# BUTSpeechFIT/huggingface_asr

Hardware: AMD Instinct MI355X
Metric: audio-seconds/sec encoder fwd+CTC, E-Branchformer-base (higher is better)
Workload: dtype bf16; 1 GPU; E-Branchformer-base enc+CTC (relative-pos), 32x10s 16kHz clips/GPU: fbank+CMVN -> conv2d sub -> 16 layers -> CTC head -> CTC loss (the batch-independent projection of the relative-position table, 0.2 % of the FLOPs, is cached across steps); per_gpu_batch=32, frames=1000, encoder_frames=250, parallelism=replicas x1 (no exchange step), steps_in_flight=4, wide_tiles=True, hw_queues=8

## Files before the change

huggingface_asr_amd/_lib.py:

```python
from __future__ import annotations

import ctypes as C
import os

_HERE = os.path.dirname(os.path.abspath(__file__))
LIB_PATH = os.environ.get("HFASR_HIP_LIB") or os.path.join(_HERE, "libhfasr_hip.so")

vp, i32, i64, f32, f64, sz = C.c_void_p, C.c_int, C.c_long, C.c_float, C.c_double, C.c_size_t


class EbfConfig(C.Structure):
    _fields_ = [(n, i32) for n in ("B", "T", "F", "d", "H", "I", "L", "V", "C1", "C2", "K", "stride", "pad",
                                   "is_causal", "pos_type", "csgu_kernel", "merge_kernel", "csgu_act", "use_macaron")] + \
               [("ln_eps", f32), ("logits_f32", i32), ("logits_ld", i32), ("branch_overlap", i32), ("extra_layers", i32), ("layer_mixing", i32), ("csgu_linear", i32),
                ("context_mode", i32), ("gate_blk", i32), ("ln_fold", i32), ("wide_tiles", i32)]


class LnRedDesc(C.Structure):
    _fields_ = [("partial", vp), ("nblk", i32), ("d", i32), ("dgamma", vp), ("dbeta", vp), ("kind", i32)]


class Gpt2Config(C.Structure):
    _fields_ = [("d", i32), ("H", i32), ("L", i32), ("V", i32), ("eps", f32), ("step_form", i32), ("act", i32)]


GLOBAL_SLOTS, LAYER_SLOTS = 24, 64

SIGNATURES = {
    "mi_gemm_bf16": [vp, i64, vp, i64, vp, i32, vp, i64, i32, vp, i64, f32, i32, i32, i32, i32, i32, i32, vp],
    "mi_conv2d_cl_bf16": [vp, vp, vp, vp] + [i32] * 13 + [vp],
    "mi_gemm_bf16_v": [vp, i64, vp, i64, vp, i32, vp, i64, i32, vp, i64, f32, i32, i32, i32, i32, i32, i32, i32, vp],
    "mi_conv2d_cl_bf16_v": [vp, vp, vp, vp] + [i32] * 14 + [vp],
    "mi_conv2d_first_gelu": [vp, vp, vp, vp] + [i32] * 10 + [vp],
    "mi_conv2d_first_geo": [vp, vp, vp, vp] + [i32] * 13 + [vp],
    "mi_conv2d_first_gated_gelu": [vp, vp, vp, vp, vp, vp] + [i32] * 10 + [vp],
    "mi_conv2d_cl_geo_bf16": [vp, vp, vp, vp] + [i32] * 15 + [vp],
    "mi_gated_act_bf16": [vp, i64, vp, i64, vp, i64, i32, i32, i32, i32, i32, i32, vp],
    "mi_im2col_cl_geo_bf16": [vp, vp] + [i32] * 12 + [vp],
    "mi_col2im_cl_bf16": [vp, vp] + [i32] * 13 + [vp],
    "mi_gated_act_bwd_bf16": [vp, i64, vp, i64, vp, i64, vp, i64, vp, i64, i32, i32, i32, i32, i32, vp],
    "mi_conv2d_first_wgrad": [vp, vp, vp, vp] + [i32] * 12 + [vp, vp],
    "mi_gemm_lnfold_bf16": [vp, i64, vp, i64, vp, vp, vp, i32, f32, vp, i64, i32, i32, i32, i32, vp],
    "mi_gemm_resid_stats_f32": [vp, i64, vp, i64, vp, vp, i64, vp, i64, f32, vp, i64, vp, i32, i32, i32, vp],
    "mi_layernorm_fold": [vp, i64, vp, i32, vp, vp, f32, vp, i64, vp, i64, vp, i32, i32, vp],
    "mi_layernorm_chain": [vp, i64, vp, i32, vp, vp, f32, vp, i64, vp, vp, f32, vp, i64, vp, i64, vp, vp, vp, i64, i32, i32, vp],
    "mi_cast_f32_bf16": [vp, i64, vp, i64, i32, i32, vp],
    "mi_rotary_bf16": [vp, i64, vp, i64, vp, vp, i32, i32, i32, i32, vp],
    "mi_attention_bf16": [vp, i64, vp, i64, vp, i64, i32, vp, i64, vp, vp, vp, vp, i64, i32, i32, i32, i32, f32, i32, vp],
    "mi_attention_qkv_bf16": [vp, i64, vp, i64, vp, i64, vp, i64, vp, vp, vp, vp, i64, i32, i32, i32, i64, i32, i32, f32, i32, vp],
    "mi_attention_qkv_bf16_v": [vp, i64, vp, i64, vp, i64, vp, i64, vp, vp, vp, vp, i64, i32, i32, i32, i64, i32, i32, f32, i32, i32, vp],
    "mi_attention_x_lse_bf16": [vp, i64, vp, i64, vp, i64, vp, vp, i64, vp, i32, i32, i32, i32, i32, f32, i32, f32, C.c_uint, C.c_uint, vp],
    "mi_attention_x_bwd_probs": [vp, i64, vp, i64, vp, i64, vp, vp, i64, vp, i64, vp, vp, vp, i64, vp, i64, i32, i32, i32, i32, i32, f32, i32, f32, C.c_uint, C.c_uint, vp],
    "mi_attention_qkv_lse_bf16": [vp, i64, vp, i64, vp, i64, vp, i64, vp, vp, vp, vp, i64, vp, i32, i32, i32, i32, f32, i32, f32, C.c_uint, C.c_uint, vp],
    "mi_attention_qkv_bwd_probs": [vp, i64, vp, i64, vp, i64, vp, i64, vp, vp, vp, vp, i64, vp, i64, vp, vp, vp, i64, vp, i64, i32,
                                   vp, i64, vp, vp, vp, vp, i64, i32, i32, i32, i32, f32, i32, f32, C.c_uint, C.c_uint, i32, vp],
    "mi_attention_qkv_bwd_fused": [vp, vp, vp, i64, vp, vp, i64, vp, i64, vp, vp, vp, vp, i64, vp, sz, i32, i32, i32, i32, f32, vp],
    "mi_row_stats_bf16": [vp, i64, i32, f32, vp, i32, vp],
    "mi_csgu_bf16": [vp, i64, vp, vp, vp, vp, vp, vp, i64, i32, i32, i32, i32, i32, i32, i32, vp],
    "mi_dwconv_residual_bf16": [vp, i64, vp, vp, vp, i64, i32, i32, i32, i32, i32, vp],
    "mi_fbank_f64": [vp, i64, vp, i32, vp, vp, vp, vp, vp, vp, i32, i32, i32, f64, f64, vp],
    "mi_trim_zeros_pad_f32": [vp, i64, vp, i32, i32, i32, vp, i64, i32, vp, vp, vp, vp],
    "mi_cmvn_utterance": [vp, vp, i32, i32, i32, i32, i32, f32, vp],
    "mi_cmvn_global": [vp, i64, i32, vp, vp, vp],
    "mi_row_lse": [vp, i64, i32, i32, vp, i32, vp],
    "mi_gemm_lse_f32": [vp, i64, vp, i64, vp, vp, i64, vp, vp, i32, i32, i32, vp],
    "mi_gemm_lse_workspace_floats": [i32, i32],
    "mi_row_argmax": [vp, i64, i32, i32, vp, i32, vp],
    "mi_ctc_collapse": [vp, i32, i32, vp, i32, i64, vp, i32, vp, vp, vp],
    "mi_ctc_greedy": [vp, i64, i64, i32, i32, i32, i32, vp, i32, i64, vp, vp, i32, vp, vp, vp],
    "mi_ctc_beam_workspace_bytes": [i32, i32, i32],
    "mi_ctc_beam_cut": [vp, i64, i64, i32, i32, i32, i32, vp, i32, i32, vp, vp, vp, vp, vp],
    "mi_ctc_beam_walk": [vp, i64, i64, i32, i32, i32, i32, vp, i32, i64, i32, i32, i32, vp, vp, vp, vp, vp, sz, vp, i32, vp, vp, vp, vp],
    "mi_ctc_beam_stream_state_bytes": [i32, i32, i32],
    "mi_ctc_beam_stream_reset": [vp, sz, i32, i32, i32, vp],
    "mi_ctc_beam_stream_walk": [vp, i64, i64, i32, i32, i32, i32, vp, i32, i64, i32, i32, i32, vp, vp, vp, vp, vp, sz, i32, i32, vp, vp, vp, vp, vp, i32, vp, vp, vp, vp],
    "mi_ctc_align_workspace_bytes": [i32, i32, i32],
    "mi_ctc_align": [vp, i64, i64, i32, vp, i32, vp, i32, vp, i32, i32, i32, vp, sz, vp, vp, vp, vp, vp, vp, vp],
    "mi_gemm_argmax_workspace_floats": [i32, i32],
    "mi_gemm_argmax_bf16": [vp, i64, vp, i64, vp, vp, vp, i32, i32, i32, vp],
    "mi_gemm_ce_f32": [vp, i64, vp, i64, vp, vp, vp, vp, vp, vp, vp, i32, i32, i32, vp],
    "mi_gemm_ce_bwd_bf16": [vp, i64, vp, i64, vp, vp, vp, vp, vp, i64, i32, i32, i32, vp],
    "mi_ctc_loss_fwd": [vp, i64, i64, i32, vp, i32, vp, i32, vp, i32, i32, i32, i32, vp, vp, vp, vp],
    "mi_ctc_prefix_prepare": [vp, i64, i64, i32, vp, i32, i32, i32, i32, i32, vp, vp, vp, vp],
    "mi_ctc_prefix_score": [vp, i32, i32, i32, i32, i32, vp, vp, i64, i32, vp, vp, vp, vp],
    "mi_embed_tokens": [vp, vp, f32, vp, i32, i32, i32, i32, i32, vp, vp],
    "mi_ce_label_smoothing": [vp, i64, vp, i32, i32, i32, i32, f32, vp, vp, vp],
    "mi_whisper_logmel": [vp, i64, vp, i32, vp, vp, vp, i32, i32, vp, vp, vp, vp],
    "mi_transpose_cast_bct_btc": [vp, vp, i32, i32, i32, vp],
    "mi_add_positions": [vp, vp, vp, i32, i32, i32, vp],
    "mi_transpose_bf16": [vp, i64, vp, i64, i32, i32, i32, vp],
    "mi_transpose_many_bf16": [vp, i32, vp],
    "mi_colsum": [vp, i64, i32, i32, i32, vp, vp, vp],
    "mi_act_fwd_bf16": [vp, i64, vp, i64, i32, i32, i32, vp],
    "mi_act_bwd_bf16": [vp, i64, vp, i64, vp, i64, i32, i32, i32, vp],
    "mi_act_dropout_fwd_bf16": [vp, i64, vp, i64, i32, i32, i32, f32, C.c_uint, C.c_uint, vp],
    "mi_act_dropout_bwd_bf16": [vp, i64, vp, i64, vp, i64, i32, i32, i32, f32, C.c_uint, C.c_uint, vp],
    "mi_layernorm_bwd_workspace_floats": [i32],
    "mi_layernorm_bwd": [vp, i64, i32, vp, f32, vp, i64, i32, vp, i64, i32, i32, vp, vp, vp, i32, i32, vp],
    "mi_layernorm_bwd_partial": [vp, i64, i32, vp, f32, vp, i64, i32, vp, i64, i32, i32, vp, vp, i32, i32, vp],
    "mi_layernorm_bwd_dual_partial": [vp, i64, i32, f32, vp, vp, i64, i32, vp, vp, i64, i32, vp, i64, i32, i32, vp, vp, vp, vp, i64, f32, f32, C.c_uint, C.c_uint, i32, i32, vp],
    "mi_layernorm_bwd_partial_cast": [vp, i64, i32, vp, f32, vp, i64, i32, vp, i64, i32, i32, vp, vp, vp, i64, f32, f32, C.c_uint, C.c_uint, i32, i32, vp],
    "mi_ln_partial_reduce_many": [vp, i32, vp],
    "mi_axpy_f32": [vp, vp, i64, f32, vp],
    "mi_scale_f32": [vp, i64, f32, vp],
    "mi_scale_dev_f32": [vp, i64, vp, vp],
    "mi_add2_cast_bf16": [vp, i64, vp, i64, vp, i64, i32, i32, f32, vp],
    "mi_add_rowvec_bf16": [vp, i64, vp, vp, i64, i32, i32, vp],
    "mi_colsum2_acc_f32": [vp, vp, i64, i32, i32, vp, vp, vp],
    "mi_colsum_cast_bf16": [vp, i64, i32, i32, vp, vp],
    "mi_add_rowvec2_bf16": [vp, i64, vp, vp, vp, vp, i64, i32, i32, vp],
    "mi_subsampled_lengths_i32": [vp, i32, i32, i32, i32, i32, i32, vp, vp, vp],
    "mi_mask_rows_f32": [vp, i64, vp, i32, i32, i32, vp],
    "mi_spec_mask_apply": [vp, i64, vp, vp, vp, i32, i32, i32, vp],
    "mi_spec_mask_bwd": [vp, i64, vp, vp, vp, i32, i32, i32, vp, vp],
    "mi_softmax_vec_f32": [vp, i32, vp, vp],
    "mi_softmax_vec_bwd_f32": [vp, vp, i32, vp, vp],
    "mi_axpy_dev_f32": [vp, vp, i64, vp, i32, vp],
    "mi_dot_f32": [vp, vp, i64, vp, vp, vp],
    "mi_sumsq_f32": [vp, i64, vp, vp, vp],
    "mi_clip_coef": [vp, f32, f32, vp, vp],
    "mi_adamw_step": [vp, vp, vp, vp, vp, i64, f32, f32, f32, f32, f32, i32, vp, vp, vp],
    "mi_gemm_tn_workspace_bytes": [i32, i32, i32],
    "mi_colsum_workspace_floats": [i32, i32],
    "mi_conv2d_first_bwd_workspace_floats": [i32, i32, i32, i32],
    "mi_conv2d_first_wgrad_workspace_floats": [i32, i32, i32, i32, i32, i32],
# ... 136 lines not shown
```

huggingface_asr_amd/csrc/conv.hip:

```cpp
#include "common.hpp"
#include "ebf_layout.hpp"

namespace {

template <int ACT>
__global__ __launch_bounds__(256) void conv2d_first_kernel(const float* __restrict__ x, const float* __restrict__ w,
                                                            const float* __restrict__ bias, bf16_t* __restrict__ out,
                                                            int B, int T, int F, int C, int KH, int KW, int st, int sf, int pad_t, int pad_f,
                                                            int T1, int F1) {
    extern __shared__ __attribute__((aligned(16))) char smem[];
    float* sw = reinterpret_cast<float*>(smem);
    float* sb = sw + KH * KW * C;
    for (int i = threadIdx.x; i < KH * KW * C; i += blockDim.x) {
        const int c = i % C, tap = i / C;
        sw[i] = w[c * KH * KW + tap];
    }
    for (int i = threadIdx.x; i < C; i += blockDim.x) sb[i] = bias[i];
    __syncthreads();
    const int cg = C >> 3;
    const long total = (long)B * T1 * F1 * cg;
    for (long idx = (long)blockIdx.x * blockDim.x + threadIdx.x; idx < total; idx += (long)gridDim.x * blockDim.x) {
        const int g = (int)(idx % cg);
        const long pos = idx / cg;
        const int f1 = (int)(pos % F1);
// ... 165 lines not shown
    }
    const int total = B * T1 * F1;
    if (pl < ppb)
    for (int pos = blockIdx.x * ppb + pl; pos < total; pos += gridDim.x * ppb) {
        const int bt = pos / F1;
        const int f1 = pos - bt * F1;
        const int b = bt / T1;
        const int t1 = bt - b * T1;
        float acc[4], gacc[4];
#pragma unroll
        for (int j = 0; j < 4; ++j) { acc[j] = br[j]; gacc[j] = gb[j]; }
        const float* xb = x + (long)b * T * F;
#pragma unroll
        for (int kh = 0; kh < 3; ++kh) {
            const int t = t1 * stride - pad_t + kh;
#pragma unroll
            for (int kw = 0; kw < 3; ++kw) {
                const int f = f1 * stride - pad_f + kw;
                const float xv = (t >= 0 && t < T && f >= 0 && f < F) ? xb[(long)t * F + f] : 0.f;
#pragma unroll
                for (int j = 0; j < 4; ++j) { acc[j] = fmaf(xv, wr[kh * 3 + kw][j], acc[j]); gacc[j] = fmaf(xv, gr[kh * 3 + kw][j], gacc[j]); }
            }
        }
        bf16x4 o;
#pragma unroll
        for (int j = 0; j < 4; ++j) o[j] = f2bf(gelu_erf(acc[j] * sigmoid_f(gacc[j])));
        *reinterpret_cast<bf16x4*>(out + (long)pos * C + g * 4) = o;
    }
}

__global__ __launch_bounds__(256) void gated_act_kernel(const bf16_t* __restrict__ z, long ldz, const bf16_t* __restrict__ g, long ldg, bf16_t* __restrict__ out, long ldo,
                                                         int B, int T, int Fq, int C, int share, int blk) {
    const int c8 = C >> 3;
    const long total = (long)B * T * Fq * c8;
    const int Tg = T / share;
    for (long i = (long)blockIdx.x * 256 + threadIdx.x; i < total; i += (long)gridDim.x * 256) {
        const int cc = (int)(i % c8) * 8;
        const long row = i / c8;
        const int f = (int)(row % Fq);
        const long bt = row / Fq;
        const int t = (int)(bt % T), b = (int)(bt / T);
        const long grow = ((long)b * Tg + t / share) * Fq + f;
        const int zc = blk ? (cc / blk) * 2 * blk + cc % blk : cc;
        const bf16x8 zv = *reinterpret_cast<const bf16x8*>(z + row * ldz + zc);
        const bf16x8 gv = *reinterpret_cast<const bf16x8*>(g + grow * ldg + (blk ? zc + blk : cc));
        bf16x8 o;
#pragma unroll
        for (int j = 0; j < 8; ++j) o[j] = f2bf(gelu_erf(bf2f(zv[j]) * sigmoid_f(bf2f(gv[j]))));
        *reinterpret_cast<bf16x8*>(out + row * ldo + cc) = o;
    }
}

__global__ __launch_bounds__(256) void row_stats_kernel(const bf16_t* __restrict__ x, long ldx, int d, float eps,
                                                         float* __restrict__ stats, int M) {
    const int lane = threadIdx.x & 63;
    const int row = blockIdx.x * 4 + (threadIdx.x >> 6);
    if (row >= M) return;
    const bf16x8* xr = reinterpret_cast<const bf16x8*>(x + (long)row * ldx);
    const int d8 = d >> 3;
    float s = 0.f, q = 0.f;
    for (int c = lane; c < d8; c += 64) {
        const bf16x8 v = xr[c];
#pragma unroll
        for (int j = 0; j < 8; ++j) s += bf2f(v[j]);
    }
    const float mean = wave_sum(s) / d;
    for (int c = lane; c < d8; c += 64) {
        const bf16x8 v = xr[c];
#pragma unroll
        for (int j = 0; j < 8; ++j) { const float a = bf2f(v[j]) - mean; q += a * a; }
    }
    const float rstd = rsqrtf(wave_sum(q) / d + eps);
    if (lane == 0) { stats[2 * row] = mean; stats[2 * row + 1] = rstd; }
}

constexpr int DW_TT = 64;
constexpr int DW_CT = 64;
constexpr int DW_KMAX = 31;

struct DwArgs {
    const bf16_t* in; long ld_in;
    const bf16_t* mul; long ld_mul;
    const float* stats;
    const float* gamma; const float* beta;
    const float* w; const float* bias;
    bf16_t* out; long ld_out;
    int B, T, C, K, pad_left, dilation, act;
};

template <bool CSGU>
__global__ __launch_bounds__(256) void dwconv_time_kernel(DwArgs p) {
    extern __shared__ __attribute__((aligned(16))) char smem[];
    const int halo = (p.K - 1) * p.dilation;
    const int rows = DW_TT + halo;
    float* tile = reinterpret_cast<float*>(smem);
    float* sw = tile + rows * DW_CT;
    const int c0 = blockIdx.x * DW_CT, t0 = blockIdx.y * DW_TT, b = blockIdx.z;
    const int tx = threadIdx.x & 63, ty = threadIdx.x >> 6;
    const int c = c0 + tx;
    const bool cok = c < p.C;
    for (int i = threadIdx.x; i < p.K * DW_CT; i += 256) {
        const int k = i / DW_CT, cc = i % DW_CT;
        sw[i] = (c0 + cc < p.C) ? p.w[(long)(c0 + cc) * p.K + k] : 0.f;
    }
    float g = 1.f, be = 0.f;
    if (CSGU && cok) { g = p.gamma[c]; be = p.beta[c]; }
    for (int r = ty; r < rows; r += 4) {
        const int t = t0 - p.pad_left + r;
        float v = 0.f;
        if (cok && t >= 0 && t < p.T) {
            const long row = (long)b * p.T + t;
            v = bf2f(p.in[row * p.ld_in + c]);
            if (CSGU) v = (v - p.stats[2 * row]) * p.stats[2 * row + 1] * g + be;
        }
        tile[r * DW_CT + tx] = v;
    }
    __syncthreads();
    if (!cok) return;
    const float bias = p.bias ? p.bias[c] : 0.f;
#pragma unroll 4
    for (int j = 0; j < DW_TT / 4; ++j) {
        const int tl = ty * (DW_TT / 4) + j;
        const int t = t0 + tl;
        if (t >= p.T) break;
        float acc = bias;
        for (int k = 0; k < p.K; ++k) acc = fmaf(sw[k * DW_CT + tx], tile[(tl + k * p.dilation) * DW_CT + tx], acc);
        const long row = (long)b * p.T + t;
        float o;
        if (CSGU) {
            if (p.act == 1) acc = gelu_erf(acc);
            else if (p.act == 2) acc = fmaxf(acc, 0.f);
            else if (p.act == 3) acc = acc / (1.f + __expf(-acc));
            o = p.mul ? bf2f(p.mul[row * p.ld_mul + c]) * acc : acc;
        } else {
            o = tile[(tl + p.pad_left) * DW_CT + tx] + acc;
        }
        p.out[row * p.ld_out + c] = f2bf(o);
    }
}

constexpr int DWF_K = 31, DWF_TT = 64, DWF_CT = 64, DWF_ROWS = DWF_TT + DWF_K - 1, DWF_PER = DWF_TT / 4;
constexpr int DWF_WS = DWF_CT + 1, DWF_WBUF = (DWF_K * DWF_WS + 3) / 4 * 4;

template <bool CSGU>
__global__ __launch_bounds__(256) void dwconv31_kernel(DwArgs p) {
    extern __shared__ __attribute__((aligned(16))) char smem[];
    float* tile = reinterpret_cast<float*>(smem);
    float* sw = tile + DWF_ROWS * DWF_CT;
    bf16_t* io = reinterpret_cast<bf16_t*>(sw + DWF_WBUF);
    const int c0 = blockIdx.x * DWF_CT, t0 = blockIdx.y * DWF_TT, b = blockIdx.z;
    const int tid = threadIdx.x;
    constexpr int NPW = (DWF_K * DWF_CT + 255) / 256;
    float wv[NPW];
#pragma unroll
    for (int q = 0; q < NPW; ++q) wv[q] = p.w[(long)c0 * DWF_K + min(tid + q * 256, DWF_K * DWF_CT - 1)];
    constexpr int NPI = (DWF_ROWS * (DWF_CT / 8) + 255) / 256, NPO = DWF_TT * (DWF_CT / 8) / 256;
    const int ch = tid & 7;
    bf16x8 vin[NPI], vio[NPO];
    float mu[NPI], rs[NPI];
    bool ok[NPI];
#pragma unroll
    for (int q = 0; q < NPI; ++q) {
        const int id = tid + q * 256, r = id >> 3;
        const int t = t0 - p.pad_left + r;
        ok[q] = id < DWF_ROWS * (DWF_CT / 8) && t >= 0 && t < p.T;
        const long row = (long)b * p.T + min(max(t, 0), p.T - 1);
        vin[q] = *reinterpret_cast<const bf16x8*>(p.in + row * p.ld_in + c0 + ch * 8);
        mu[q] = 0.f; rs[q] = 0.f;
        if (CSGU) { mu[q] = p.stats[2 * row]; rs[q] = p.stats[2 * row + 1]; }
    }
    f32x4 g0 = {1.f, 1.f, 1.f, 1.f}, g1 = g0, b0 = {0.f, 0.f, 0.f, 0.f}, b1 = b0;
    if (CSGU) {
        g0 = *reinterpret_cast<const f32x4*>(p.gamma + c0 + ch * 8); g1 = *reinterpret_cast<const f32x4*>(p.gamma + c0 + ch * 8 + 4);
        b0 = *reinterpret_cast<const f32x4*>(p.beta + c0 + ch * 8);  b1 = *reinterpret_cast<const f32x4*>(p.beta + c0 + ch * 8 + 4);
#pragma unroll
        for (int q = 0; q < NPO; ++q) {
            const int r = (tid + q * 256) >> 3, t = t0 + r;
            vio[q] = *reinterpret_cast<const bf16x8*>(p.mul + ((long)b * p.T + min(t, p.T - 1)) * p.ld_mul + c0 + ch * 8);
        }
    }
    __builtin_amdgcn_sched_barrier(0);
#pragma unroll
    for (int q = 0; q < NPW; ++q) {
        const int i = tid + q * 256;
        if (i < DWF_K * DWF_CT) sw[(i % DWF_K) * DWF_WS + i / DWF_K] = wv[q];
    }
#pragma unroll
    for (int q = 0; q < NPI; ++q) {
        const int id = tid + q * 256, r = id >> 3;
        if (id < DWF_ROWS * (DWF_CT / 8)) {
            f32x4 lo = {0.f, 0.f, 0.f, 0.f}, hi = {0.f, 0.f, 0.f, 0.f};
            if (ok[q]) {
                float f[8];
#pragma unroll
                for (int j = 0; j < 8; ++j) f[j] = bf2f(vin[q][j]);
                if (CSGU) {
                    lo = f32x4{(f[0] - mu[q]) * rs[q] * g0.x + b0.x, (f[1] - mu[q]) * rs[q] * g0.y + b0.y, (f[2] - mu[q]) * rs[q] * g0.z + b0.z, (f[3] - mu[q]) * rs[q] * g0.w + b0.w};
                    hi = f32x4{(f[4] - mu[q]) * rs[q] * g1.x + b1.x, (f[5] - mu[q]) * rs[q] * g1.y + b1.y, (f[6] - mu[q]) * rs[q] * g1.z + b1.z, (f[7] - mu[q]) * rs[q] * g1.w + b1.w};
                } else {
                    lo = f32x4{f[0], f[1], f[2], f[3]};
                    hi = f32x4{f[4], f[5], f[6], f[7]};
                }
            }
            *reinterpret_cast<f32x4*>(tile + r * DWF_CT + ch * 8) = lo;
            *reinterpret_cast<f32x4*>(tile + r * DWF_CT + ch * 8 + 4) = hi;
        }
    }
    if (CSGU) {
#pragma unroll
        for (int q = 0; q < NPO; ++q) {
            const int r = (tid + q * 256) >> 3;
            *reinterpret_cast<bf16x8*>(io + r * DWF_CT + ch * 8) = vio[q];
        }
    }
    __syncthreads();
    const int tx = tid & 63, ty = tid >> 6;
    const int c = c0 + tx;
    float wk[DWF_K];
#pragma unroll
    for (int k = 0; k < DWF_K; ++k) wk[k] = sw[k * DWF_WS + tx];
    float win[DWF_PER + DWF_K - 1];
#pragma unroll
    for (int i = 0; i < DWF_PER + DWF_K - 1; ++i) win[i] = tile[(ty * DWF_PER + i) * DWF_CT + tx];
    const float bias = p.bias ? p.bias[c] : 0.f;
#pragma unroll
    for (int j = 0; j < DWF_PER; ++j) {
        float acc = bias;
#pragma unroll
        for (int k = 0; k < DWF_K; ++k) acc = fmaf(wk[k], win[j + k], acc);
        const int rl = ty * DWF_PER + j;
        float o;
        if (CSGU) {
            if (p.act == 1) acc = gelu_erf(acc);
            else if (p.act == 2) acc = fmaxf(acc, 0.f);
            else if (p.act == 3) acc = acc / (1.f + __expf(-acc));
            o = bf2f(io[rl * DWF_CT + tx]) * acc;
        } else {
            o = win[j + (DWF_K - 1) / 2] + acc;
        }
        io[rl * DWF_CT + tx] = f2bf(o);
    }
    __syncthreads();
    for (int id = tid; id < DWF_TT * (DWF_CT / 8); id += 256) {
        const int r = id >> 3, ch = id & 7;
        const int t = t0 + r;
        if (t < p.T)
            *reinterpret_cast<bf16x8*>(p.out + ((long)b * p.T + t) * p.ld_out + c0 + ch * 8) = *reinterpret_cast<const bf16x8*>(io + r * DWF_CT + ch * 8);
    }
}

}

extern "C" int mi_conv2d_first_gelu(const float* x, const float* w, const float* bias, void* out_cl_bf16,
                                    int B, int T, int F, int C, int K, int stride, int pad_t, int pad_f,
                                    int T1, int F1, hipStream_t stream) {
    MI_ENTER();
    if (B <= 0 || T <= 0 || F <= 0 || C <= 0 || (C % 8) != 0 || K <= 0 || K > 7) return MI_ERR_ARG;
    const int cgs = C / 8;
    if (K == 3 && C == 256 && (long)B * T1 * F1 < (1L << 31) - (1L << 20) && (reinterpret_cast<uintptr_t>(out_cl_bf16) & 15) == 0) {
        const long ntiles = ((long)B * T1 * F1 + 31) / 32;
        const long nb = (ntiles + 3) / 4;
        hipLaunchKernelGGL(conv2d_first3_mfma_kernel, dim3((unsigned)(nb < 2048 ? nb : 2048)), dim3(256), 4 * 32 * 256 * 2, stream, x, w, bias, (bf16_t*)out_cl_bf16,
                           B, T, F, stride, pad_t, pad_f, T1, F1);
        MI_CHECK_LAUNCH();
        return MI_OK;
    }
    if (K == 3 && cgs <= 256 && (256 % cgs) == 0 && (long)B * T1 * F1 < (1L << 31) - 256L * 8192) {
        const long npos = (long)B * T1 * F1;
        const int ppb = 256 / cgs;
        const long nb = (npos + ppb - 1) / ppb;
        hipLaunchKernelGGL(conv2d_first3_kernel, dim3((unsigned)(nb < 8192 ? nb : 8192)), dim3(256), 0, stream, x, w, bias,
                           (bf16_t*)out_cl_bf16, B, T, F, C, stride, pad_t, pad_f, T1, F1);
        MI_CHECK_LAUNCH();
        return MI_OK;
    }
    const long total = (long)B * T1 * F1 * (C / 8);
    const int grid = (int)((total + 255) / 256 < 4096 ? (total + 255) / 256 : 4096);
    const size_t lds = (size_t)(K * K * C + C) * sizeof(float);
    hipLaunchKernelGGL(conv2d_first_kernel<1>, dim3(grid), dim3(256), lds, stream, x, w, bias, (bf16_t*)out_cl_bf16,
                       B, T, F, C, K, K, stride, stride, pad_t, pad_f, T1, F1);
    MI_CHECK_LAUNCH();
    return MI_OK;
}

extern "C" int mi_conv2d_first_geo(const float* x, const float* w, const float* bias, void* out_cl_bf16, int B, int T, int F, int C,
                                   int KH, int KW, int stride_t, int stride_f, int pad_t, int pad_f, int T1, int F1, int act, hipStream_t stream) {
    MI_ENTER();
    if (B <= 0 || T <= 0 || F <= 0 || C <= 0 || (C % 8) != 0 || KH <= 0 || KW <= 0 || KH * KW > 64 || stride_t <= 0 || stride_f <= 0 || T1 <= 0 || F1 <= 0) return MI_ERR_ARG;
    if ((T1 - 1) * stride_t - pad_t >= T || (F1 - 1) * stride_f - pad_f >= F) return MI_ERR_ARG;
    const size_t lds = (size_t)(KH * KW * C + C) * sizeof(float);
    if (lds > 64 * 1024) return MI_ERR_UNSUPPORTED;
    const long total = (long)B * T1 * F1 * (C / 8);
    const int grid = (int)((total + 255) / 256 < 4096 ? (total + 255) / 256 : 4096);
    if (act) hipLaunchKernelGGL(conv2d_first_kernel<1>, dim3(grid), dim3(256), lds, stream, x, w, bias, (bf16_t*)out_cl_bf16, B, T, F, C, KH, KW, stride_t, stride_f, pad_t, pad_f, T1, F1);
    else hipLaunchKernelGGL(conv2d_first_kernel<0>, dim3(grid), dim3(256), lds, stream, x, w, bias, (bf16_t*)out_cl_bf16, B, T, F, C, KH, KW, stride_t, stride_f, pad_t, pad_f, T1, F1);
    MI_CHECK_LAUNCH();
    return MI_OK;
}

extern "C" int mi_conv2d_first_gated_gelu(const float* x, const float* w, const float* bias, const float* gw, const float* gbias, void* out_cl_bf16,
                                          int B, int T, int F, int C, int K, int stride, int pad_t, int pad_f, int T1, int F1, hipStream_t stream) {
    MI_ENTER();
    if (B <= 0 || T <= 0 || F <= 0 || C <= 0 || T1 <= 0 || F1 <= 0) return MI_ERR_ARG;
    if (!conv1_gated_fused(B, T1, F1, C, K)) return MI_ERR_UNSUPPORTED;
    const int cgs = C / 4;
    const long npos = (long)B * T1 * F1;
    const int ppb = 256 / cgs;
    const long nb = (npos + ppb - 1) / ppb;
    hipLaunchKernelGGL(conv2d_first3_gated_kernel, dim3((unsigned)(nb < 8192 ? nb : 8192)), dim3(256), 0, stream, x, w, bias, gw, gbias,
                       (bf16_t*)out_cl_bf16, B, T, F, C, stride, pad_t, pad_f, T1, F1);
    MI_CHECK_LAUNCH();
    return MI_OK;
}

extern "C" int mi_gated_act_bf16(const void* z, long ldz, const void* g, long ldg, void* out, long ldo, int B, int T, int Fq, int C, int share, int blk,
                                 hipStream_t stream) {
    MI_ENTER();
    auto al16 = [](const void* q) { return (reinterpret_cast<uintptr_t>(q) & 15) == 0; };
    if (B <= 0 || T <= 0 || Fq <= 0 || C <= 0 || (C % 8) != 0 || share <= 0 || (T % share) != 0 || blk < 0 || (blk && ((blk % 8) != 0 || (C % blk) != 0))) return MI_ERR_ARG;
    if ((ldz % 8) || (ldg % 8) || (ldo % 8) || !al16(z) || !al16(g) || !al16(out)) return MI_ERR_ARG;
    const long blocks = ((long)B * T * Fq * (C / 8) + 255) / 256;
    hipLaunchKernelGGL(gated_act_kernel, dim3((unsigned)(blocks < 16384 ? blocks : 16384)), dim3(256), 0, stream, (const bf16_t*)z, ldz, (const bf16_t*)g, ldg,
                       (bf16_t*)out, ldo, B, T, Fq, C, share, blk);
    MI_CHECK_LAUNCH();
    return MI_OK;
}

extern "C" int mi_row_stats_bf16(const void* x, long ldx, int d, float eps, float* stats, int M, hipStream_t stream) {
    MI_ENTER();
    if (M <= 0 || d <= 0 || (d % 8) != 0 || (ldx % 8) != 0) return MI_ERR_ARG;
    hipLaunchKernelGGL(row_stats_kernel, dim3(cdiv(M, 4)), dim3(256), 0, stream, (const bf16_t*)x, ldx, d, eps, stats, M);
    MI_CHECK_LAUNCH();
    return MI_OK;
}

static int dw_launch(const DwArgs& a, bool csgu, hipStream_t stream) {
    if (a.B <= 0 || a.T <= 0 || a.C <= 0 || a.K <= 0 || a.K > DW_KMAX || a.dilation < 1) return MI_ERR_ARG;
    const int halo = (a.K - 1) * a.dilation;
    const size_t lds = (size_t)((DW_TT + halo) * DW_CT + a.K * DW_CT) * sizeof(float);
    if (lds > 160 * 1024) return MI_ERR_UNSUPPORTED;
    const bool fast = !(csgu && !a.mul) && a.K == DWF_K && a.dilation == 1 && a.pad_left == (DWF_K - 1) / 2 && (a.C % DWF_CT) == 0 &&
                      (a.ld_in % 8) == 0 && (((uintptr_t)a.in) & 15) == 0 && (a.ld_out % 8) == 0 && (((uintptr_t)a.out) & 15) == 0 &&
                      (!csgu || ((a.ld_mul % 8) == 0 && (((uintptr_t)a.mul) & 15) == 0)) && (!csgu || (((uintptr_t)a.gamma | (uintptr_t)a.beta) & 15) == 0);
    if (fast) {
        dim3 gridf(a.C / DWF_CT, cdiv(a.T, DWF_TT), a.B);
        const size_t ldsf = (size_t)(DWF_ROWS * DWF_CT + DWF_WBUF) * sizeof(float) + (size_t)DWF_TT * DWF_CT * sizeof(bf16_t);
        if (csgu) hipLaunchKernelGGL(dwconv31_kernel<true>, gridf, dim3(256), ldsf, stream, a);
        else hipLaunchKernelGGL(dwconv31_kernel<false>, gridf, dim3(256), ldsf, stream, a);
        MI_CHECK_LAUNCH();
        return MI_OK;
    }
    dim3 grid(cdiv(a.C, DW_CT), cdiv(a.T, DW_TT), a.B);
    if (csgu) hipLaunchKernelGGL(dwconv_time_kernel<true>, grid, dim3(256), lds, stream, a);
    else hipLaunchKernelGGL(dwconv_time_kernel<false>, grid, dim3(256), lds, stream, a);
    MI_CHECK_LAUNCH();
    return MI_OK;
}

extern "C" int mi_csgu_bf16(const void* u, long ldu, const float* stats, const float* gamma, const float* beta,
                            const float* w, const float* bias, void* out, long ldo,
                            int B, int T, int C, int K, int pad_left, int dilation, int act, hipStream_t stream) {
    MI_ENTER();
    DwArgs a{};
    a.in = (const bf16_t*)u + C; a.ld_in = ldu; a.mul = (const bf16_t*)u; a.ld_mul = ldu; a.stats = stats;
    a.gamma = gamma; a.beta = beta; a.w = w; a.bias = bias; a.out = (bf16_t*)out; a.ld_out = ldo;
    a.B = B; a.T = T; a.C = C; a.K = K; a.pad_left = pad_left; a.dilation = dilation; a.act = act;
    return dw_launch(a, true, stream);
}

extern "C" int mi_csgu_conv_bf16(const void* u, long ldu, const float* stats, const float* gamma, const float* beta,
                                 const float* w, const float* bias, void* out, long ldo,
                                 int B, int T, int C, int K, int pad_left, int dilation, hipStream_t stream) {
    MI_ENTER();
    DwArgs a{};
    a.in = (const bf16_t*)u + C; a.ld_in = ldu; a.mul = nullptr; a.ld_mul = 0; a.stats = stats;
    a.gamma = gamma; a.beta = beta; a.w = w; a.bias = bias; a.out = (bf16_t*)out; a.ld_out = ldo;
    a.B = B; a.T = T; a.C = C; a.K = K; a.pad_left = pad_left; a.dilation = dilation; a.act = 0;
    return dw_launch(a, true, stream);
}

__global__ __launch_bounds__(256) void gate_act_mul_kernel(const bf16_t* r, long ldr, const bf16_t* g, long ldg, bf16_t* out, long ldo, long M, int C, int act) {
    const long n = M * C;
    for (long i = (long)blockIdx.x * 256 + threadIdx.x; i < n; i += (long)gridDim.x * 256) {
        const long row = i / C;
        const int c = (int)(i - row * C);
        float v = bf2f(g[row * ldg + c]);
        if (act == 1) v = gelu_erf(v);
        else if (act == 2) v = fmaxf(v, 0.f);
        else if (act == 3) v = v / (1.f + __expf(-v));
        out[row * ldo + c] = f2bf(bf2f(r[row * ldr + c]) * v);
    }
}

extern "C" int mi_gate_act_mul_bf16(const void* r, long ldr, const void* g, long ldg, void* out, long ldo, long M, int C, int act, hipStream_t stream) {
    MI_ENTER();
    if (M <= 0 || C <= 0 || act < 0 || act > 3) return MI_ERR_ARG;
    const long blocks = (M * C + 255) / 256;
    hipLaunchKernelGGL(gate_act_mul_kernel, dim3((unsigned)(blocks < 8192 ? blocks : 8192)), dim3(256), 0, stream,
                       (const bf16_t*)r, ldr, (const bf16_t*)g, ldg, (bf16_t*)out, ldo, M, C, act);
    MI_CHECK_LAUNCH();
    return MI_OK;
}

extern "C" int mi_dwconv_residual_bf16(const void* m, long ldm, const float* w, const float* bias, void* out, long ldo,
                                       int B, int T, int C, int K, int pad_left, hipStream_t stream) {
    MI_ENTER();
    DwArgs a{};
    a.in = (const bf16_t*)m; a.ld_in = ldm; a.w = w; a.bias = bias; a.out = (bf16_t*)out; a.ld_out = ldo;
    a.B = B; a.T = T; a.C = C; a.K = K; a.pad_left = pad_left; a.dilation = 1; a.act = 0;
    return dw_launch(a, false, stream);
}
```

huggingface_asr_amd/csrc/encoder.hip:

```cpp
#include "ebf_layout.hpp"

namespace {

struct Ws {
    bf16_t *act1, *act2, *a0, *a1, *a2, *a1r, *h, *qk, *vt, *ctx, *cat, *m2, *s, *hid;
    bf16_t *cv, *lin;
    bf16_t *z1, *g1, *z2, *g2;
    float *feo, *x, *stats, *lnst;
    float *mixed, *lh, *sw;
    int* lens;
    size_t bytes;
};

Ws carve(const mi_ebf_config& c, const Dims& d, void* base) {
    Carver k{(char*)base, 0};
    auto bf = [&](size_t n) { return (bf16_t*)k.take(n * 2); };
    auto f32 = [&](size_t n) { return (float*)k.take(n * 4); };
    Ws w;
    const size_t M = d.M, dd = c.d, I = c.I, n1 = (size_t)c.B * d.T1 * d.F1 * c.C1, n2 = (size_t)c.B * d.T2 * d.F2 * c.C2;
    w.act1 = bf(n1); w.act2 = bf(n2);
    w.z1 = w.g1 = w.z2 = w.g2 = nullptr;
    if (c.context_mode == 1) {
        if (!conv1_gated_fused(c.B, d.T1, d.F1, c.C1, c.K)) { w.z1 = bf(n1); w.g1 = bf(n1); }
        w.z2 = bf(2 * n2);
    } else if (c.context_mode == 2) {
        w.z1 = bf(n1); w.g1 = bf((size_t)c.B * (d.T1 / 4 + 1) * d.F1 * c.C1);
        w.z2 = bf(n2); w.g2 = bf((size_t)c.B * (d.T2 / 4 + 1) * d.F2 * c.C2);
    }
    w.feo = f32(M * dd); w.x = f32(M * dd);
    w.a0 = bf(M * dd); w.a1 = bf(M * dd); w.a2 = bf(M * dd); w.a1r = bf(M * dd);
    w.h = bf(M * I);
    w.qk = bf(M * 3 * dd);
    w.vt = bf(dd * c.B * d.Tp);
    w.ctx = bf(M * dd); w.cat = bf(M * 2 * dd); w.m2 = bf(M * 2 * dd); w.s = bf(M * (I / 2));
    w.cv = w.lin = nullptr;
    if (c.csgu_linear) { w.cv = bf(M * (I / 2)); w.lin = bf(M * (I / 2)); }
    w.hid = bf(M * dd);
    w.stats = f32(M * 2);
    w.lnst = c.ln_fold ? f32(M * 32) : nullptr;
    w.lens = (int*)k.take((size_t)2 * c.B * 4);
    w.mixed = w.lh = w.sw = nullptr;
    if (c.layer_mixing) { w.mixed = f32(M * dd); w.sw = f32((size_t)(c.L + 1)); }
    if (c.layer_mixing || c.extra_layers) w.lh = f32(M * dd);
    w.bytes = k.off;
    return w;
}

__device__ __forceinline__ int floor_div(int a, int d) { int q = a / d; if ((a % d) != 0 && ((a < 0) != (d < 0))) --q; return q; }
__global__ void subsampled_lengths_kernel(const int* __restrict__ in, int T, int B, int K, int stride, int pad_total, int layers, int tmax,
                                          int* __restrict__ inner, int* __restrict__ outer) {
    const int b = blockIdx.x * blockDim.x + threadIdx.x;
    if (b >= B) return;
    int li = in ? in[b] : T, lo = li;
    for (int i = 0; i < layers; ++i) { li = floor_div(li + pad_total - K, stride) + 1; lo = floor_div(lo - K, stride) + 1; }
    inner[b] = li < tmax ? li : tmax;
    outer[b] = lo;
}

constexpr int MAX_OVL_LAYERS = 64;
hipStream_t g_side = nullptr;
hipEvent_t g_fork[MAX_OVL_LAYERS], g_join[MAX_OVL_LAYERS];
bool side_ready() {
    if (g_side) return true;
    if (hipStreamCreateWithFlags(&g_side, hipStreamNonBlocking) != hipSuccess) { g_side = nullptr; return false; }
    for (int i = 0; i < MAX_OVL_LAYERS; ++i)
        if (hipEventCreateWithFlags(&g_fork[i], hipEventDisableTiming) != hipSuccess || hipEventCreateWithFlags(&g_join[i], hipEventDisableTiming) != hipSuccess) {
            g_side = nullptr;
            return false;
        }
    return true;
}

constexpr float LEPS = 1e-5f;

struct Fwd : Slots {
    const mi_ebf_config& c; const Dims D; const Ws w; hipStream_t st;
    const int* mask_len;
    const void* pos_table; void* posp;
    const int M, d, I, T2, P;
    const int dil, cpad;
    const float scale;
    Fwd(const mi_ebf_config& c_, const Dims& D_, const Ws& w_, const void* const* weights, hipStream_t st_, const int* mask, const void* pos_table_, void* posp_)
        : Slots{weights}, c(c_), D(D_), w(w_), st(st_), mask_len(mask), pos_table(pos_table_), posp(posp_), M(D_.M), d(c_.d), I(c_.I), T2(D_.T2), P(2 * D_.T2 - 1),
          dil(c_.is_causal ? (c_.csgu_kernel - 1) / 2 : 1), cpad(c_.is_causal ? (c_.csgu_kernel - 1) * dil : (c_.csgu_kernel - 1) / 2), scale(1.0f / sqrtf((float)D_.hd)) {}

    const bf16_t* posp_of(int l) const { return c.pos_type == 1 ? (const bf16_t*)posp + (size_t)l * P * d : nullptr; }
    const float* pos_u(int l) const { return c.pos_type == 1 ? Lf(l, ATT_U) : nullptr; }
    const float* pos_v(int l) const { return c.pos_type == 1 ? Lf(l, ATT_V) : nullptr; }
    int keep_hidden(float* hidden_states, int l, const float* src) const {
        if (hidden_states && hipMemcpyAsync(hidden_states + (size_t)l * M * d, src, (size_t)M * d * sizeof(float), hipMemcpyDeviceToDevice, st) != hipSuccess) return MI_ERR_LAUNCH;
        return MI_OK;
    }
    int front_end(const float* feats) const;
    int enter_layer(const float* src, int l) const;
    int project_positions(int layers) const;
    int attention_qkv(int l) const;
    int local_gate(int l, hipStream_t sl) const;
    int merge_dwconv(int l) const;
    int plain_layer(int l, int Lt) const;
    int folded_layer(int l) const;
    int encoder_exit(int l, float* last_hidden) const;
    int ctc_head(void* logits, float* lse, float* lse_workspace, int* best, float* amax_workspace) const;
};

int Fwd::front_end(const float* feats) const {
    const int pl = c.is_causal ? 2 * c.pad : c.pad;
    if (c.context_mode < 0 || c.context_mode > 2 || (c.context_mode && c.is_causal)) return MI_ERR_ARG;
    if (c.context_mode == 0) {
        RUN(mi_conv2d_first_gelu(feats, Gf(G_CONV1_W), Gf(G_CONV1_B), w.act1, c.B, c.T, c.F, c.C1, c.K, c.stride, pl, pl, D.T1, D.F1, st));
        RUN(mi_conv2d_cl_bf16(w.act1, Gw(G_CONV2_W), Gf(G_CONV2_B), w.act2, c.B, D.T1, D.F1, c.C1, c.C2, c.K, c.K, c.stride, pl, pl,
                              D.T2, D.F2, 1, st));
    } else if (c.context_mode == 1) {
        if (c.gate_blk <= 0 || (c.C2 % c.gate_blk) != 0) return MI_ERR_ARG;
        int rc = mi_conv2d_first_gated_gelu(feats, Gf(G_CONV1_W), Gf(G_CONV1_B), Gf(G_GATE1_W), Gf(G_GATE1_B), w.act1, c.B, c.T, c.F, c.C1, c.K, c.stride, pl, pl, D.T1, D.F1, st);
        if (rc == MI_ERR_UNSUPPORTED) {
            RUN(mi_conv2d_first_geo(feats, Gf(G_CONV1_W), Gf(G_CONV1_B), w.z1, c.B, c.T, c.F, c.C1, c.K, c.K, c.stride, c.stride, pl, pl, D.T1, D.F1, 0, st));
            RUN(mi_conv2d_first_geo(feats, Gf(G_GATE1_W), Gf(G_GATE1_B), w.g1, c.B, c.T, c.F, c.C1, c.K, c.K, c.stride, c.stride, pl, pl, D.T1, D.F1, 0, st));
            RUN(mi_gated_act_bf16(w.z1, c.C1, w.g1, c.C1, w.act1, c.C1, c.B, D.T1, D.F1, c.C1, 1, 0, st));
        } else if (rc != MI_OK) return rc;
        rc = c.gate_blk == 32 ? mi_conv2d_cl_geo_bf16(w.act1, Gw(G_CONV2_W), Gf(G_CONV2_B), w.act2, c.B, D.T1, D.F1, c.C1, c.C2, c.K, c.K, c.stride, c.stride, pl, pl, D.T2, D.F2, 1, 1, st)
                              : MI_ERR_UNSUPPORTED;
        if (rc == MI_ERR_UNSUPPORTED) {
            RUN(mi_conv2d_cl_geo_bf16(w.act1, Gw(G_CONV2_W), Gf(G_CONV2_B), w.z2, c.B, D.T1, D.F1, c.C1, 2 * c.C2, c.K, c.K, c.stride, c.stride, pl, pl, D.T2, D.F2, 0, 0, st));
            RUN(mi_gated_act_bf16(w.z2, 2 * c.C2, w.z2, 2 * c.C2, w.act2, c.C2, c.B, D.T2, D.F2, c.C2, 1, c.gate_blk, st));
        } else if (rc != MI_OK) return rc;
    } else {
        const int KH = 4 * c.K, sg = 4 * c.stride, pg = 4 * c.pad;
        const int Tg1 = conv_out(c.T, KH, sg, 2 * pg), Tg2 = conv_out(D.T1, KH, sg, 2 * pg);
        if ((D.T1 % 4) != 0 || Tg1 != D.T1 / 4 || (D.T2 % 4) != 0 || Tg2 != D.T2 / 4) return MI_ERR_ARG;
        RUN(mi_conv2d_first_geo(feats, Gf(G_CONV1_W), Gf(G_CONV1_B), w.z1, c.B, c.T, c.F, c.C1, c.K, c.K, c.stride, c.stride, pl, pl, D.T1, D.F1, 0, st));
        RUN(mi_conv2d_first_geo(feats, Gf(G_GATE1_W), Gf(G_GATE1_B), w.g1, c.B, c.T, c.F, c.C1, KH, c.K, sg, c.stride, pg, pl, Tg1, D.F1, 0, st));
        RUN(mi_gated_act_bf16(w.z1, c.C1, w.g1, c.C1, w.act1, c.C1, c.B, D.T1, D.F1, c.C1, 4, 0, st));
        RUN(mi_conv2d_cl_bf16(w.act1, Gw(G_CONV2_W), Gf(G_CONV2_B), w.z2, c.B, D.T1, D.F1, c.C1, c.C2, c.K, c.K, c.stride, pl, pl, D.T2, D.F2, 0, st));
        RUN(mi_conv2d_cl_geo_bf16(w.act1, Gw(G_GATE2_W), Gf(G_GATE2_B), w.g2, c.B, D.T1, D.F1, c.C1, c.C2, KH, c.K, sg, c.stride, pg, pl, Tg2, D.F2, 0, 0, st));
        RUN(mi_gated_act_bf16(w.z2, c.C2, w.g2, c.C2, w.act2, c.C2, c.B, D.T2, D.F2, c.C2, 4, 0, st));
    }
    const int gv = c.wide_tiles ? 40 : 0;
    auto linear = [&](const bf16_t* A, long K, const void* W, const float* bias, float* C) {
        int rc = gv ? mi_gemm_bf16_v(A, K, W, K, bias, 1, C, d, 1, nullptr, 0, 1.f, 0, M, d, (int)K, 0, 0, gv, st) : MI_ERR_UNSUPPORTED;
        if (rc == MI_ERR_UNSUPPORTED) rc = mi_gemm_bf16(A, K, W, K, bias, 1, C, d, 1, nullptr, 0, 1.f, 0, M, d, (int)K, 0, 0, st);
        return rc;
    };
    RUN(linear(w.act2, (long)D.F2 * c.C2, Gw(G_FEOUT_W), Gf(G_FEOUT_B), w.feo));
    RUN(mi_layernorm_chain(w.feo, d, nullptr, T2, nullptr, nullptr, 0.f, nullptr, 0, Gf(G_FP_LN_G), Gf(G_FP_LN_B), c.ln_eps,
                           w.a0, d, nullptr, 0, nullptr, nullptr, nullptr, 0, M, d, st));
    return linear(w.a0, d, Gw(G_FP_W), Gf(G_FP_B), w.x);
}

int Fwd::enter_layer(const float* src, int l) const {
    if (c.use_macaron)
        return mi_layernorm_chain(src, d, mask_len, T2, nullptr, nullptr, 0.f, w.x, d, Lf(l, FF1_LN_G), Lf(l, FF1_LN_B), LEPS,
                                  w.a0, d, nullptr, 0, nullptr, nullptr, nullptr, 0, M, d, st);
    return mi_layernorm_chain(src, d, mask_len, T2, nullptr, nullptr, 0.f, w.x, d, Lf(l, ATT_LN_G), Lf(l, ATT_LN_B), LEPS,
                              w.a1, d, nullptr, 0, Lf(l, MLP_LN_G), Lf(l, MLP_LN_B), w.a2, d, M, d, st);
}

int Fwd::project_positions(int layers) const {
    for (int l = 0; l < layers; ++l)
        RUN(mi_gemm_bf16(pos_table, d, Lw(l, ATT_WPOS), d, nullptr, 0, (bf16_t*)posp + (size_t)l * P * d, d, 0, nullptr, 0, 1.f, 0,
                         P, d, d, 0, 0, st));
    return MI_OK;
}

int Fwd::attention_qkv(int l) const {
    return mi_attention_qkv_bf16(w.qk, 3 * d, w.qk + d, 3 * d, w.qk + 2 * d, 3 * d, posp_of(l), d, pos_u(l), pos_v(l),
                                 mask_len, w.ctx, d, c.B, T2, 0, 0, c.H, D.hd, scale, c.is_causal, st);
}

int Fwd::local_gate(int l, hipStream_t sl) const {
    const int kc = c.csgu_kernel;
    RUN(mi_row_stats_bf16(w.h + I / 2, I, I / 2, LEPS, w.stats, M, sl));
    if (!c.csgu_linear)
        return mi_csgu_bf16(w.h, I, w.stats, Lf(l, CSGU_LN_G), Lf(l, CSGU_LN_B), Lf(l, CSGU_W), Lf(l, CSGU_B), w.s, I / 2, c.B, T2, I / 2, kc, cpad, dil, c.csgu_act, sl);
    RUN(mi_csgu_conv_bf16(w.h, I, w.stats, Lf(l, CSGU_LN_G), Lf(l, CSGU_LN_B), Lf(l, CSGU_W), Lf(l, CSGU_B), w.cv, I / 2, c.B, T2, I / 2, kc, cpad, dil, sl));
    RUN(mi_gemm_bf16(w.cv, I / 2, Lw(l, CSGU_LIN_W), I / 2, Lf(l, CSGU_LIN_B), 1, w.lin, I / 2, 0, nullptr, 0, 1.f, 0, M, I / 2, I / 2, 0, 0, sl));
    return mi_gate_act_mul_bf16(w.h, I, w.lin, I / 2, w.s, I / 2, M, I / 2, c.csgu_act, sl);
}

int Fwd::merge_dwconv(int l) const {
    const int km = c.merge_kernel;
    return mi_dwconv_residual_bf16(w.cat, 2 * d, Lf(l, MRG_DW_W), Lf(l, MRG_DW_B), w.m2, 2 * d, c.B, T2, 2 * d, km, (km - 1) / 2, st);
}

int Fwd::plain_layer(int l, int Lt) const {
    if (c.layer_mixing && l < c.L) RUN(mi_axpy_dev_f32(w.mixed, w.x, (long)M * d, w.sw + l, l == 0, st));
    if (c.use_macaron) {
        RUN(mi_gemm_bf16(w.a0, d, Lw(l, FF1_W1), d, Lf(l, FF1_B1), 1, w.h, I, 0, nullptr, 0, 1.f, 1, M, I, d, 0, 0, st));
        RUN(mi_gemm_bf16(w.h, I, Lw(l, FF1_W2), I, Lf(l, FF1_B2), 1, w.x, d, 1, w.x, d, 0.5f, 0, M, d, I, 0, 0, st));
        RUN(mi_layernorm_chain(w.x, d, nullptr, T2, nullptr, nullptr, 0.f, nullptr, 0, Lf(l, ATT_LN_G), Lf(l, ATT_LN_B), LEPS,
                               w.a1, d, nullptr, 0, Lf(l, MLP_LN_G), Lf(l, MLP_LN_B), w.a2, d, M, d, st));
    }
    const bool ovl = c.branch_overlap && l < MAX_OVL_LAYERS && side_ready();
    hipStream_t sl = ovl ? g_side : st;
    if (ovl) { (void)hipEventRecord(g_fork[l], st); (void)hipStreamWaitEvent(g_side, g_fork[l], 0); }
    const bf16_t* qk_in = w.a1;
    if (c.pos_type == 2) {
        const float* rot_cos = (const float*)pos_table;
        RUN(mi_rotary_bf16(w.a1, d, w.a1r, d, rot_cos, rot_cos ? rot_cos + (size_t)T2 * D.hd : nullptr, M, T2, c.H, D.hd, st));
        qk_in = w.a1r;
    }
    if (D.hd == 64 || D.hd == 128) {
        if (c.pos_type == 2) {
            RUN(mi_gemm_bf16(qk_in, d, Lw(l, ATT_WQK), d, Lf(l, ATT_BQK), 1, w.qk, 3 * d, 0, nullptr, 0, 1.f, 0, M, 2 * d, d, 0, 0, st));
            RUN(mi_gemm_bf16(w.a1, d, Lw(l, ATT_WV), d, Lf(l, ATT_BV), 1, w.qk + 2 * d, 3 * d, 0, nullptr, 0, 1.f, 0, M, d, d, 0, 0, st));
        } else {
            RUN(mi_gemm_bf16(w.a1, d, Lw(l, ATT_WQK), d, Lf(l, ATT_BQK), 1, w.qk, 3 * d, 0, nullptr, 0, 1.f, 0, M, 3 * d, d, 0, 0, st));
        }
        RUN(attention_qkv(l));
    } else {
        RUN(mi_gemm_bf16(qk_in, d, Lw(l, ATT_WQK), d, Lf(l, ATT_BQK), 1, w.qk, 3 * d, 0, nullptr, 0, 1.f, 0, M, 2 * d, d, 0, 0, st));
        RUN(mi_gemm_bf16(Lw(l, ATT_WV), d, w.a1, d, Lf(l, ATT_BV), 2, w.vt, (long)c.B * D.Tp, 0, nullptr, 0, 1.f, 0, d, M, d,
                         T2, D.Tp, st));
        RUN(mi_attention_bf16(w.qk, 3 * d, w.qk + d, 3 * d, w.vt, (long)c.B * D.Tp, D.Tp, posp_of(l), d, pos_u(l), pos_v(l),
                              mask_len, w.ctx, d, c.B, T2, c.H, D.hd, scale, c.is_causal, st));
    }
    RUN(mi_gemm_bf16(w.ctx, d, Lw(l, ATT_WO), d, Lf(l, ATT_BO), 1, w.cat, 2 * d, 0, nullptr, 0, 1.f, 0, M, d, d, 0, 0, st));
    RUN(mi_gemm_bf16(w.a2, d, Lw(l, MLP_W1), d, Lf(l, MLP_B1), 1, w.h, I, 0, nullptr, 0, 1.f, 1, M, I, d, 0, 0, sl));
    RUN(local_gate(l, sl));
    RUN(mi_gemm_bf16(w.s, I / 2, Lw(l, MLP_W2), I / 2, Lf(l, MLP_B2), 1, w.cat + d, 2 * d, 0, nullptr, 0, 1.f, 0, M, d, I / 2, 0, 0, sl));
    if (ovl) { (void)hipEventRecord(g_join[l], g_side); (void)hipStreamWaitEvent(st, g_join[l], 0); }
    RUN(merge_dwconv(l));
    RUN(mi_gemm_bf16(w.m2, 2 * d, Lw(l, MRG_W), 2 * d, Lf(l, MRG_B), 1, w.x, d, 1, w.x, d, 1.0f, 0, M, d, 2 * d, 0, 0, st));
    if (c.use_macaron) {
        RUN(mi_layernorm_chain(w.x, d, nullptr, T2, nullptr, nullptr, 0.f, nullptr, 0, Lf(l, FF2_LN_G), Lf(l, FF2_LN_B), LEPS,
                               w.a0, d, nullptr, 0, nullptr, nullptr, nullptr, 0, M, d, st));
        RUN(mi_gemm_bf16(w.a0, d, Lw(l, FF2_W1), d, Lf(l, FF2_B1), 1, w.h, I, 0, nullptr, 0, 1.f, 1, M, I, d, 0, 0, st));
        RUN(mi_gemm_bf16(w.h, I, Lw(l, FF2_W2), I, Lf(l, FF2_B2), 1, w.x, d, 1, w.x, d, 0.5f, 0, M, d, I, 0, 0, st));
    }
    if (l + 1 == c.L) return MI_OK;
    if (l + 1 == Lt)
        return mi_layernorm_chain(w.x, d, nullptr, T2, nullptr, nullptr, 0.f, nullptr, 0, Lf(l, FIN_LN_G), Lf(l, FIN_LN_B), LEPS,
                                  w.hid, d, nullptr, 0, nullptr, nullptr, nullptr, 0, M, d, st);
    if (c.use_macaron)
        return mi_layernorm_chain(w.x, d, nullptr, T2, Lf(l, FIN_LN_G), Lf(l, FIN_LN_B), LEPS, w.x, d,
                                  Lf(l + 1, FF1_LN_G), Lf(l + 1, FF1_LN_B), LEPS, w.a0, d, nullptr, 0, nullptr, nullptr, nullptr, 0, M, d, st);
    return mi_layernorm_chain(w.x, d, nullptr, T2, Lf(l, FIN_LN_G), Lf(l, FIN_LN_B), LEPS, w.x, d,
                              Lf(l + 1, ATT_LN_G), Lf(l + 1, ATT_LN_B), LEPS, w.a1, d, nullptr, 0,
                              Lf(l + 1, MLP_LN_G), Lf(l + 1, MLP_LN_B), w.a2, d, M, d, st);
}

int Fwd::folded_layer(int l) const {
    const int gv = c.wide_tiles ? 40 : 0;
    const int npg = c.wide_tiles ? d / 64 : d / 32;
    RUN(mi_gemm_lnfold_bf16(w.a0, d, Lw(l, FF1_WF), d, Lf(l, FF1_SF), Lf(l, FF1_CF), w.lnst, 1, LEPS, w.h, I, 1, M, I, d, st));
    RUN(mi_gemm_resid_stats_f32_v(w.h, I, Lw(l, FF1_W2), I, Lf(l, FF1_B2), w.x, d, w.x, d, 0.5f, w.a0, d, w.lnst, M, d, I, gv, st));
    RUN(mi_gemm_lnfold_bf16(w.a0, d, Lw(l, QKV_WF), d, Lf(l, QKV_SF), Lf(l, QKV_CF), w.lnst, npg, LEPS, w.qk, 3 * d, 0, M, 3 * d, d, st));
    RUN(attention_qkv(l));
    RUN(mi_gemm_bf16_v(w.ctx, d, Lw(l, ATT_WO), d, Lf(l, ATT_BO), 1, w.cat, 2 * d, 0, nullptr, 0, 1.f, 0, M, d, d, 0, 0, gv, st));
    RUN(mi_gemm_lnfold_bf16(w.a0, d, Lw(l, MLP_WF), d, Lf(l, MLP_SF), Lf(l, MLP_CF), w.lnst, npg, LEPS, w.h, I, 1, M, I, d, st));
    RUN(local_gate(l, st));
    RUN(mi_gemm_bf16_v(w.s, I / 2, Lw(l, MLP_W2), I / 2, Lf(l, MLP_B2), 1, w.cat + d, 2 * d, 0, nullptr, 0, 1.f, 0, M, d, I / 2, 0, 0, gv, st));
    RUN(merge_dwconv(l));
    RUN(mi_gemm_resid_stats_f32_v(w.m2, 2 * d, Lw(l, MRG_W), 2 * d, Lf(l, MRG_B), w.x, d, w.x, d, 1.0f, w.a0, d, w.lnst, M, d, 2 * d, gv, st));
    RUN(mi_gemm_lnfold_bf16(w.a0, d, Lw(l, FF2_WF), d, Lf(l, FF2_SF), Lf(l, FF2_CF), w.lnst, npg, LEPS, w.h, I, 1, M, I, d, st));
    RUN(mi_gemm_bf16_v(w.h, I, Lw(l, FF2_W2), I, Lf(l, FF2_B2), 1, w.x, d, 1, w.x, d, 0.5f, 0, M, d, I, 0, 0, gv, st));
    if (l + 1 == c.L) return MI_OK;
    return mi_layernorm_fold(w.x, d, nullptr, T2, Lf(l, FIN_LN_G), Lf(l, FIN_LN_B), LEPS, w.x, d, w.a0, d, w.lnst, M, d, st);
}

int Fwd::encoder_exit(int l, float* last_hidden) const {
    const bool tune = c.layer_mixing || c.extra_layers;
    float* lh = (last_hidden || !tune) ? last_hidden : w.lh;
    RUN(mi_layernorm_chain(w.x, d, nullptr, T2, Lf(l, FIN_LN_G), Lf(l, FIN_LN_B), LEPS, nullptr, 0,
                           Gf(G_ENC_LN_G), Gf(G_ENC_LN_B), c.ln_eps, w.hid, d, lh, d, nullptr, nullptr, nullptr, 0, M, d, st));
    if (!tune) return MI_OK;
    const float* top = lh;
    if (c.layer_mixing) {
        RUN(mi_axpy_dev_f32(w.mixed, lh, (long)M * d, w.sw + c.L, 0, st));
        top = w.mixed;
    }
    return c.extra_layers ? enter_layer(top, c.L) : mi_add2_cast_bf16(top, d, nullptr, 0, w.hid, d, M, d, 1.f, st);
}

int Fwd::ctc_head(void* logits, float* lse, float* lse_workspace, int* best, float* amax_workspace) const {
    if (!best && !logits) return MI_OK;
    const long ldl = c.logits_ld > 0 ? c.logits_ld : c.V + 1;
    int rc = MI_ERR_UNSUPPORTED;
    if (best && amax_workspace) rc = mi_gemm_argmax_bf16(w.hid, d, Gw(G_HEAD_W), d, Gf(G_HEAD_B), best, amax_workspace, M, c.V + 1, d, st);
    else if (!best && lse) rc = mi_gemm_lse_f32(w.hid, d, Gw(G_HEAD_W), d, Gf(G_HEAD_B), (float*)logits, ldl, lse, lse_workspace, M, c.V + 1, d, st);
    if (rc != MI_ERR_UNSUPPORTED) return rc;
    if (!logits) return MI_ERR_UNSUPPORTED;
    RUN(mi_gemm_bf16(w.hid, d, Gw(G_HEAD_W), d, Gf(G_HEAD_B), 1, logits, ldl, c.logits_f32, nullptr, 0, 1.f, 0, M, c.V + 1, d, 0, 0, st));
    if (best) return mi_row_argmax(logits, ldl, c.logits_f32 ? 0 : 1, c.V + 1, best, M, st);
    return lse ? mi_row_lse(logits, ldl, 0, c.V + 1, lse, M, st) : MI_OK;
}

}

void launch_subsampled_lengths(const int* lengths, int T, int B, int K, int stride, int pad_total, int layers, int tmax, int* inner, int* outer, hipStream_t st) {
    hipLaunchKernelGGL(subsampled_lengths_kernel, dim3(cdiv(B, 64)), dim3(64), 0, st, lengths, T, B, K, stride, pad_total, layers, tmax, inner, outer);
}

extern "C" size_t mi_ebf_workspace_bytes(const mi_ebf_config* cfg) { return sizable(cfg) ? carve(*cfg, dims(*cfg), nullptr).bytes : 0; }

extern "C" int mi_gemm_lse_f32(const void* A, long lda, const void* W, long ldw, const float* bias, float* C, long ldc, float* lse, float* workspace,
                               int M, int N, int K, hipStream_t stream);
extern "C" int mi_row_lse(const void* x, long ld, int dtype, int V, float* lse, int M, hipStream_t stream);
static int ebf_forward_body(const mi_ebf_config* cfg, const void* const* weights, const float* feats, const int* feat_lengths, const void* pos_table, void* posp, int compute_posp,
                            void* workspace, size_t workspace_bytes, float* last_hidden, void* logits, int* inner_len, int* outer_len, float* hidden_states,
                            float* lse, float* lse_workspace, int* best, float* amax_workspace, hipStream_t st) {
    if (!cfg || cfg->H <= 0) return MI_ERR_ARG;
    MI_ENTER();
    const mi_ebf_config& c = *cfg;
    if ((lse != nullptr) != (lse_workspace != nullptr) || (lse && (!logits || !c.logits_f32))) return MI_ERR_ARG;
    if (hidden_states && !last_hidden) return MI_ERR_ARG;
    if (best && !amax_workspace && !logits) return MI_ERR_ARG;
    if (best && !logits && ((c.d % 64) != 0 || c.d < 128)) return MI_ERR_UNSUPPORTED;
    if (c.B <= 0 || c.T <= 0 || c.L <= 0 || c.d % c.H || c.I % 2) return MI_ERR_ARG;
    if (c.extra_layers < 0 || c.extra_layers > 1 || (c.layer_mixing && c.L + 1 > 1024)) return MI_ERR_ARG;
    const int Lt = c.L + c.extra_layers;
    const Dims D = dims(c);
    if (D.T2 <= 0) return MI_ERR_ARG;
    const Ws w = carve(c, D, workspace);
    if (w.bytes > workspace_bytes) return MI_ERR_ARG;
    int* inner = inner_len ? inner_len : w.lens;
    int* outer = outer_len ? outer_len : w.lens + c.B;
    launch_subsampled_lengths(feat_lengths, c.T, c.B, c.K, c.stride, c.is_causal ? c.K - 1 : 2 * c.pad, 2, D.T2, inner, outer, st);
    const Fwd f(c, D, w, weights, st, feat_lengths ? inner : nullptr, pos_table, posp);

    RUN(f.front_end(feats));
    if (!c.ln_fold) RUN(f.enter_layer(w.x, 0));
    if (c.layer_mixing) RUN(mi_softmax_vec_f32(f.Gf(G_MIX_W), c.L + 1, w.sw, st));
    if (c.pos_type == 1 && compute_posp) RUN(f.project_positions(Lt));
    if (c.ln_fold) {
        if (c.pos_type == 2 || !c.use_macaron || c.extra_layers || c.layer_mixing || c.csgu_linear || (D.hd != 64 && D.hd != 128)) return MI_ERR_ARG;
        RUN(mi_layernorm_fold(w.x, c.d, f.mask_len, D.T2, nullptr, nullptr, 0.f, w.x, c.d, w.a0, c.d, w.lnst, D.M, c.d, st));
    }
    for (int l = 0; l < Lt; ++l) {
        if (l < c.L) RUN(f.keep_hidden(hidden_states, l, w.x));
        RUN(c.ln_fold ? f.folded_layer(l) : f.plain_layer(l, Lt));
        if (l + 1 == c.L) RUN(f.encoder_exit(l, last_hidden));
    }
    RUN(f.ctc_head(logits, lse, lse_workspace, best, amax_workspace));
// ... 30 lines not shown
```

huggingface_asr_amd/csrc/gemm_8p.hip:

```cpp
#include "gemm_args.hpp"
#include <type_traits>

#ifndef GEMM_FLOOR
#define GEMM_FLOOR 0
#endif
#ifndef GEMM128_LOADER
#define GEMM128_LOADER 0
#endif

namespace {

typedef __attribute__((address_space(1))) const void* gptr_t;
typedef __attribute__((address_space(3))) void* lptr_t;

constexpr int TB = 256, BK = 64;
constexpr int BUF = 65536, BOFF = 32768;

template <int N>
__device__ __forceinline__ void wait_vm() {
    if constexpr (N >= 0) asm volatile("s_waitcnt vmcnt(%0)" ::"n"(N) : "memory");
}
__device__ __forceinline__ void barrier() {
    __builtin_amdgcn_sched_barrier(0);
    asm volatile("s_barrier" ::: "memory");
    __builtin_amdgcn_sched_barrier(0);
}
__device__ __forceinline__ void wait_lds() {
    asm volatile("s_waitcnt lgkmcnt(0)" ::: "memory");
    __builtin_amdgcn_sched_barrier(0);
}

__device__ __attribute__((aligned(16))) uint4 g_zero_page8p = {0u, 0u, 0u, 0u};

struct Ctx {
    const char* A; const char* W;
    unsigned offA[2][2], offB[2][2];
    int cti[2][2], cfi[2][2];
    unsigned dA[2][2], dB[2][2];
    unsigned aRd[2], bRd[2];
};

template <bool CONV, int ACT, bool OUT32 = false, bool GATED = false, bool LNF = false, bool LSE = false, bool AMAX = false, int CE = 0>
__global__ __launch_bounds__(512, 2) void gemm8p_kernel(GemmArgs p) {
    extern __shared__ __attribute__((aligned(16))) char smem[];
    const int tid = threadIdx.x, lane = tid & 63;
    const int wave = __builtin_amdgcn_readfirstlane(tid >> 6);
    const int wr = wave >> 2, wc = wave & 3;

    const int ntm = (p.M + TB - 1) / TB, ntn = (p.N + TB - 1) / TB;
    const int nwg = ntm * ntn;
    int bid = blockIdx.x;
    {
        const int q = nwg >> 3, r = nwg & 7, xcd = bid & 7, idx = bid >> 3;
        bid = (xcd < r ? xcd * (q + 1) : r * (q + 1) + (xcd - r) * q) + idx;
    }
    const int m0 = (bid / ntn) * TB, n0 = (bid % ntn) * TB;

    Ctx c;
    c.A = reinterpret_cast<const char*>(p.A);
    c.W = reinterpret_cast<const char*>(p.W);
    {
        const int prow = lane >> 3, pc = lane & 7;
#pragma unroll
        for (int h = 0; h < 2; ++h)
#pragma unroll
            for (int e = 0; e < 2; ++e) {
                const int ra = wr * 128 + h * 64 + (2 * wc + e) * 8;
                const int rb = (wave >> 1) * 64 + h * 32 + (2 * (wave & 1) + e) * 8;
                const int lcA = pc ^ (((ra + prow) >> 1) & 7), lcB = pc ^ (((rb + prow) >> 1) & 7);
                if constexpr (CONV) {
                    const int m = min(m0 + ra + prow, p.M - 1);
                    const int fo = m % p.Fout, to = (m / p.Fout) % p.Tout, b = m / (p.Fout * p.Tout);
                    c.cti[h][e] = to * p.stride - p.pad_t;
                    c.cfi[h][e] = fo * p.stride_f - p.pad_f;
                    c.offA[h][e] = (unsigned)b * (unsigned)(p.Tin * p.Fin * p.Cin * 2) + lcA * 16;
                } else {
                    c.offA[h][e] = (unsigned)min(m0 + ra + prow, p.M - 1) * (unsigned)(p.lda * 2) + lcA * 16;
                }
                c.offB[h][e] = (unsigned)min(n0 + rb + prow, p.N - 1) * (unsigned)(p.ldw * 2) + lcB * 16;
                c.dA[h][e] = ra * 128;
                c.dB[h][e] = BOFF + rb * 128;
            }
        const int fr = lane & 15, fq = lane >> 4, swz = (fr >> 1) & 7;
        const unsigned low = fr * 128 + ((fq ^ swz) << 4);
        c.aRd[0] = wr * 128 * 128 + low;
        c.aRd[1] = c.aRd[0] ^ 64;
        c.bRd[0] = BOFF + wc * 64 * 128 + low;
        c.bRd[1] = c.bRd[0] ^ 64;
    }
    auto stageA = [&](int kt, unsigned buf, int mq) {
        if (GEMM_FLOOR == 2) return;
        if constexpr (CONV) {
            const int ntap = p.K / p.Cin;
            const int chunk = kt / ntap, tap = kt - chunk * ntap, c0 = chunk * BK;
            const int kh = tap / p.KW, kw = tap - kh * p.KW;
#pragma unroll
            for (int e = 0; e < 2; ++e) {
                const int ti = c.cti[mq][e] + kh, fi = c.cfi[mq][e] + kw;
                const bool ok = (unsigned)ti < (unsigned)p.Tin && (unsigned)fi < (unsigned)p.Fin;
                const char* sp = ok ? c.A + (c.offA[mq][e] + (unsigned)(((ti * p.Fin + fi) * p.Cin + c0) * 2)) : reinterpret_cast<const char*>(&g_zero_page8p);
                __builtin_amdgcn_global_load_lds((gptr_t)sp, (lptr_t)(smem + buf + c.dA[mq][e]), 16, 0, 0);
            }
        } else {
#pragma unroll
            for (int e = 0; e < 2; ++e)
                __builtin_amdgcn_global_load_lds((gptr_t)(c.A + c.offA[mq][e] + (unsigned)kt * 128u), (lptr_t)(smem + buf + c.dA[mq][e]), 16, 0, 0);
        }
    };
    auto conv_k = [&](int kt) { const int ntap = p.K / p.Cin; const int chunk = kt / ntap; return (kt - chunk * ntap) * p.Cin + chunk * BK; };
    auto stageB = [&](int kt, unsigned buf, int nq) {
        if (GEMM_FLOOR == 2) return;
        const unsigned kb = CONV ? (unsigned)conv_k(kt) * 2u : (unsigned)kt * 128u;
#pragma unroll
        for (int e = 0; e < 2; ++e)
            __builtin_amdgcn_global_load_lds((gptr_t)(c.W + c.offB[nq][e] + kb), (lptr_t)(smem + buf + c.dB[nq][e]), 16, 0, 0);
    };

    f32x4 acc[8][4];
#pragma unroll
    for (int i = 0; i < 8; ++i)
#pragma unroll
        for (int j = 0; j < 4; ++j) acc[i][j] = f32x4{0.f, 0.f, 0.f, 0.f};
    bf16x8 fa[4][2], fb[2][2][2];

    auto readA = [&](unsigned cb, int mq) {
// ... 262 lines not shown
                const int m = m0 + wr * 128 + row;
                if (m < p.M) *reinterpret_cast<uint4*>(C + (long)m * p.ldc + ob + c4 * 8) = v;
            }
        }
        return;
    }
    if constexpr (ACT >= 3) {
        const bool drop = p.drop_p > 0.f;
        const float inv_keep = drop ? 1.f / (1.f - p.drop_p) : 1.f;
        const int n8 = p.N >> 3;
#pragma unroll
        for (int blk = 0; blk < 4; ++blk) {
            bf16x8 ax[4];
            if constexpr (ACT == 3) {
#pragma unroll
                for (int uu = 0; uu < 4; ++uu) {
                    const int m = m0 + wr * 128 + (blk * 4 + uu) * 8 + prow;
                    ax[uu] = *reinterpret_cast<const bf16x8*>(p.aux + (long)min(m, p.M - 1) * p.ldaux + nb + pc * 8);
                }
            }
#pragma unroll
            for (int ii = 0; ii < 2; ++ii) {
                const int i = blk * 2 + ii;
#pragma unroll
                for (int j = 0; j < 4; ++j) {
                    const f32x4 v = acc[i][j] + b4[j];
                    const bf16x4 o = {f2bf(v.x), f2bf(v.y), f2bf(v.z), f2bf(v.w)};
                    const int row = i * 16 + fr;
                    *reinterpret_cast<bf16x4*>(reg + row * 128 + (((j * 2 + (fq >> 1)) ^ swz) << 4) + (fq & 1) * 8) = o;
                }
            }
            asm volatile("s_waitcnt lgkmcnt(0)" ::: "memory");
#pragma unroll
            for (int uu = 0; uu < 4; ++uu) {
                const int row = (blk * 4 + uu) * 8 + prow;
                const bf16x8 v = *reinterpret_cast<const bf16x8*>(reg + row * 128 + ((pc ^ ((row >> 1) & 7)) << 4));
                const int m = m0 + wr * 128 + row;
                float ks[8];
                if (drop) {
                    const unsigned long long quad0 = ((unsigned long long)m * n8 + ((nb >> 3) + pc)) << 1;
                    mask_keep4(p.drop_key, quad0, p.drop_p, inv_keep, ks);
                    mask_keep4(p.drop_key, quad0 + 1, p.drop_p, inv_keep, ks + 4);
                }
                bf16x8 o;
                if constexpr (ACT == 3) {
                    float gr[8];
                    if (p.aux_kind == 1) {
#pragma unroll
                        for (int e = 0; e < 8; ++e) gr[e] = gelu_erf_grad(bf2f(ax[uu][e]));
                    } else {
#pragma unroll
                        for (int e = 0; e < 8; ++e) gr[e] = gelu_tanh_grad(bf2f(ax[uu][e]));
                    }
#pragma unroll
                    for (int e = 0; e < 8; ++e) {
                        const float g = drop ? bf2f(f2bf(bf2f(v[e]) * ks[e])) : bf2f(v[e]);
                        o[e] = f2bf(g * gr[e]);
                    }
                    if (m < p.M) *reinterpret_cast<bf16x8*>(C + (long)m * p.ldc + nb + pc * 8) = o;
                } else {
                    float ac[8];
                    if (p.aux_kind == 1) {
#pragma unroll
                        for (int e = 0; e < 8; ++e) ac[e] = gelu_erf(bf2f(v[e]));
                    } else {
#pragma unroll
                        for (int e = 0; e < 8; ++e) ac[e] = gelu_tanh(bf2f(v[e]));
                    }
#pragma unroll
                    for (int e = 0; e < 8; ++e) {
                        bf16_t r = f2bf(ac[e]);
                        if (drop) r = f2bf(bf2f(r) * ks[e]);
                        o[e] = r;
                    }
                    if (m < p.M) {
                        *reinterpret_cast<bf16x8*>(C + (long)m * p.ldc + nb + pc * 8) = v;
                        *reinterpret_cast<bf16x8*>(p.C2 + (long)m * p.ldc2 + nb + pc * 8) = o;
                    }
                }
            }
        }
        return;
    }
#pragma unroll
    for (int blk = 0; blk < 4; ++blk) {
#pragma unroll
        for (int ii = 0; ii < 2; ++ii) {
            const int i = blk * 2 + ii;
#pragma unroll
            for (int j = 0; j < 4; ++j) {
                f32x4 v = acc[i][j] + b4[j];
                if constexpr (ACT == 1) v = f32x4{gelu_erf(v.x), gelu_erf(v.y), gelu_erf(v.z), gelu_erf(v.w)};
                else if constexpr (ACT == 2) v = f32x4{gelu_tanh(v.x), gelu_tanh(v.y), gelu_tanh(v.z), gelu_tanh(v.w)};
                const bf16x4 o = {f2bf(v.x), f2bf(v.y), f2bf(v.z), f2bf(v.w)};
                const int row = i * 16 + fr;
                *reinterpret_cast<bf16x4*>(reg + row * 128 + (((j * 2 + (fq >> 1)) ^ swz) << 4) + (fq & 1) * 8) = o;
            }
        }
        asm volatile("s_waitcnt lgkmcnt(0)" ::: "memory");
#pragma unroll
        for (int u = blk * 4; u < blk * 4 + 4; ++u) {
            const int row = u * 8 + prow;
            const uint4 v = *reinterpret_cast<const uint4*>(reg + row * 128 + ((pc ^ ((row >> 1) & 7)) << 4));
            const int m = m0 + wr * 128 + row;
            if (m < p.M) *reinterpret_cast<uint4*>(C + (long)m * p.ldc + nb + pc * 8) = v;
        }
    }
}

constexpr int B128_BUF = 32768, B128_BOFF = 16384;

template <int NB>
__global__ __launch_bounds__(512, 2) void gemm8p128_kernel(GemmArgs p) {
    extern __shared__ __attribute__((aligned(16))) char smem[];
    const int tid = threadIdx.x, lane = tid & 63;
    const int wave = __builtin_amdgcn_readfirstlane(tid >> 6);
    const int wr = wave >> 2, wc = wave & 3;

    const int ntm = (p.M + 127) / 128, ntn = p.N / 128;
    const int nwg = ntm * ntn;
    int bid = blockIdx.x;
    {
        const int q = nwg >> 3, r = nwg & 7, xcd = bid & 7, idx = bid >> 3;
        bid = (xcd < r ? xcd * (q + 1) : r * (q + 1) + (xcd - r) * q) + idx;
    }
    const int m0 = (bid / ntn) * 128, n0 = (bid % ntn) * 128;
    const int prow = lane >> 3, pc = lane & 7;

    const int nb = n0 + wc * 32;
    f32x4 rres[8];
    const bool use_res = p.out_f32 && p.resid != nullptr;
    if (use_res) {
#pragma unroll
        for (int u = 0; u < 8; ++u) {
            const int m = min(m0 + wr * 64 + u * 8 + prow, p.M - 1);
            rres[u] = *reinterpret_cast<const f32x4*>(p.resid + (long)m * p.ldr + nb + pc * 4);
        }
    }

    const char* src_base = reinterpret_cast<const char*>(wave < 4 ? (const void*)p.A : (const void*)p.W);
    unsigned off[4], dst[4];
#pragma unroll
    for (int e = 0; e < 4; ++e) {
        const int r0 = (4 * (wave & 3) + e) * 8;
        const int lc = pc ^ (((r0 + prow) >> 1) & 7);
        if (wave < 4) off[e] = (unsigned)min(m0 + r0 + prow, p.M - 1) * (unsigned)(p.lda * 2) + lc * 16;
        else off[e] = (unsigned)min(n0 + r0 + prow, p.N - 1) * (unsigned)(p.ldw * 2) + lc * 16;
        dst[e] = (wave < 4 ? 0 : B128_BOFF) + r0 * 128;
    }
    auto stage = [&](int kt) {
        const unsigned buf = (unsigned)(NB == 4 ? (kt & 3) : kt % NB) * B128_BUF;
#pragma unroll
        for (int e = 0; e < 4; ++e)
            __builtin_amdgcn_global_load_lds((gptr_t)(src_base + off[e] + (unsigned)kt * 128u), (lptr_t)(smem + buf + dst[e]), 16, 0, 0);
    };
    const int fr = lane & 15, fq = lane >> 4, swz = (fr >> 1) & 7;
    const unsigned low = fr * 128 + ((fq ^ swz) << 4);
    const unsigned aRd0 = wr * 64 * 128 + low, bRd0 = B128_BOFF + wc * 32 * 128 + low;

    f32x4 acc[4][2];
#pragma unroll
    for (int i = 0; i < 4; ++i)
#pragma unroll
        for (int j = 0; j < 2; ++j) acc[i][j] = f32x4{0.f, 0.f, 0.f, 0.f};
    bf16x8 fa[4][2], fb[2][2];
    auto phase = [&](int kt, auto DO_STAGE, auto WAIT) {
        const unsigned cb = (unsigned)(NB == 4 ? (kt & 3) : kt % NB) * B128_BUF;
#pragma unroll
        for (int j = 0; j < 2; ++j)
#pragma unroll
            for (int s = 0; s < 2; ++s) fb[j][s] = *reinterpret_cast<const bf16x8*>(smem + ((cb + bRd0) ^ (s * 64)) + j * 16 * 128);
#pragma unroll
        for (int i = 0; i < 4; ++i)
#pragma unroll
            for (int s = 0; s < 2; ++s) fa[i][s] = *reinterpret_cast<const bf16x8*>(smem + ((cb + aRd0) ^ (s * 64)) + i * 16 * 128);
        if constexpr (decltype(DO_STAGE)::value) stage(kt + NB - 1);
        wait_vm<decltype(WAIT)::value>();
        wait_lds();
        barrier();
        __builtin_amdgcn_s_setprio(1);
#pragma unroll
        for (int s = 0; s < 2; ++s)
#pragma unroll
            for (int i = 0; i < 4; ++i)
#pragma unroll
                for (int j = 0; j < 2; ++j)
                    acc[i][j] = __builtin_amdgcn_mfma_f32_16x16x32_bf16(fb[j][s], fa[i][s], acc[i][j], 0, 0, 0);
        __builtin_amdgcn_s_setprio(0);
// ... 438 lines not shown
    }

    if (wave < 4) {
#pragma unroll
        for (int j = 0; j < 4; ++j) {
            const int nb = n0 + wc * 64 + j * 16 + fq * 4;
            const f32x4 b4 = (p.bias_mode == 1) ? *reinterpret_cast<const f32x4*>(p.bias + nb) : f32x4{0.f, 0.f, 0.f, 0.f};
#pragma unroll
            for (int i = 0; i < 4; ++i) {
                f32x4 v = acc[i][j] + b4;
                if (p.act == 1) v = f32x4{gelu_erf(v.x), gelu_erf(v.y), gelu_erf(v.z), gelu_erf(v.w)};
                else if (p.act == 2) v = f32x4{gelu_tanh(v.x), gelu_tanh(v.y), gelu_tanh(v.z), gelu_tanh(v.w)};
                const int row = wr * 64 + i * 16 + fr;
                const int ch = wc * 16 + j * 4 + fq;
                *reinterpret_cast<f32x4*>(smem + row * 512 + ((ch ^ (row & 31)) << 4)) = v;
            }
        }
    }
    __syncthreads();
    if (p.out_f32) {
        float* C = reinterpret_cast<float*>(p.C);
#pragma unroll
        for (int u = 0; u < 8; ++u) {
            const int row = wave * 16 + u * 2 + er;
            f32x4 v = *reinterpret_cast<const f32x4*>(smem + row * 512 + ((ec ^ (row & 31)) << 4));
            const int m = m0 + row, n = n0 + ec * 4;
            if (p.drop_p > 0.f) {
                float k4[4];
                mask_keep4(p.drop_key, (unsigned long long)m * (unsigned)(p.N >> 2) + (unsigned)(n >> 2), p.drop_p, 1.f / (1.f - p.drop_p), k4);
                v = f32x4{v.x * k4[0], v.y * k4[1], v.z * k4[2], v.w * k4[3]};
            }
            if (use_res) v = rres[u] + p.alpha * v;
            if (m < p.M) *reinterpret_cast<f32x4*>(C + (long)m * p.ldc + n) = v;
            if (p.C2 && m < p.M) *reinterpret_cast<bf16x4*>(p.C2 + (long)m * p.ldc2 + n) = bf16x4{f2bf(v.x), f2bf(v.y), f2bf(v.z), f2bf(v.w)};
            if (p.stats_out) {
                float sm = (v.x + v.y) + (v.z + v.w), sq = (v.x * v.x + v.y * v.y) + (v.z * v.z + v.w * v.w);
                sm += dpp_f32<0xB1, 0xF>(0.f, sm); sq += dpp_f32<0xB1, 0xF>(0.f, sq);
                sm += dpp_f32<0x4E, 0xF>(0.f, sm); sq += dpp_f32<0x4E, 0xF>(0.f, sq);
                sm += dpp_f32<0x141, 0xF>(0.f, sm); sq += dpp_f32<0x141, 0xF>(0.f, sq);
                if ((ec & 7) == 0 && m < p.M) *reinterpret_cast<f32x2*>(p.stats_out + (long)m * LN_STATS_STRIDE + (((n0 >> 7) << 2) + (ec >> 3)) * 2) = f32x2{sm, sq};
            }
        }
    } else {
        bf16_t* C = reinterpret_cast<bf16_t*>(p.C);
#pragma unroll
        for (int u = 0; u < 8; ++u) {
            const int row = wave * 16 + u * 2 + er;
            const f32x4 v = *reinterpret_cast<const f32x4*>(smem + row * 512 + ((ec ^ (row & 31)) << 4));
            const int m = m0 + row, n = n0 + ec * 4;
            bf16x4 o = {f2bf(v.x), f2bf(v.y), f2bf(v.z), f2bf(v.w)};
            if (p.drop_p > 0.f) {
                float k4[4];
                mask_keep4(p.drop_key, ((unsigned long long)m * (unsigned)p.N + (unsigned)n) >> 2, p.drop_p, 1.f / (1.f - p.drop_p), k4);
#pragma unroll
                for (int q = 0; q < 4; ++q) o[q] = f2bf(bf2f(o[q]) * k4[q]);
            }
            if (m < p.M) *reinterpret_cast<bf16x4*>(C + (long)m * p.ldc + n) = o;
        }
    }
}

}

bool gemm_8p_supported(const GemmArgs& a, bool conv) {
    if (a.M <= 0 || a.N <= 0 || (a.K % BK) != 0 || a.K < 2 * BK) return false;
    if (a.col_T || a.bias_mode == 2) return false;
    if (a.resid && (!a.out_f32 || (a.N % TB) != 0 || ((uintptr_t)a.resid & 15) || (a.ldr % 4) != 0)) return false;
    if (((uintptr_t)a.A & 15) || ((uintptr_t)a.W & 15) || ((uintptr_t)a.C & 15) || (a.ldw % 8)) return false;
    if (a.out_f32) {
        if (conv || a.act != 0 || (a.ldc % 4) != 0 || a.ldc < ((a.N + 3) & ~3)) return false;
    } else {
        if ((a.N % TB) != 0 || (a.ldc % 8) != 0) return false;
        if (a.bias_mode == 1 && ((uintptr_t)a.bias & 15)) return false;
    }
    if (a.gated && (!conv || a.out_f32 || a.act != 1)) return false;
    if (a.ln_stats) {
        if (conv || a.out_f32 || a.gated || a.act > 1 || a.bias_mode != 1 || !a.ln_colsum || ((uintptr_t)a.ln_colsum & 15) || ((uintptr_t)a.ln_stats & 15)) return false;
        if (!(a.ln_npart == 1 || (a.ln_npart >= 4 && a.ln_npart <= 16 && (a.ln_npart % 4) == 0))) return false;
    }
    if (a.act >= 3) {
        if (conv || a.out_f32 || a.gated || a.ln_stats || a.resid || a.col_T || a.act > 4 || (a.aux_kind != 1 && a.aux_kind != 2) || a.drop_p < 0.f || a.drop_p >= 1.f) return false;
        if (a.act == 3 && (!a.aux || ((uintptr_t)a.aux & 15) || (a.ldaux % 8))) return false;
        if (a.act == 4 && (!a.C2 || ((uintptr_t)a.C2 & 15) || (a.ldc2 % 8))) return false;
    } else if (a.C2 || a.stats_out) {
        if (!a.out_f32 || !a.resid || a.N > 1024 || (a.C2 && (((uintptr_t)a.C2 & 7) || (a.ldc2 % 4))) || ((uintptr_t)a.stats_out & 7)) return false;
    }
    if (a.lse_part && (conv || !a.out_f32 || a.resid || a.C2 || a.stats_out || a.act != 0 || ((uintptr_t)a.lse_part & 7) || (a.lse_ld % 2) || a.lse_ld < 8 * cdiv(a.N, TB))) return false;
    if (a.amax_part && (conv || !a.out_f32 || a.resid || a.C2 || a.stats_out || a.lse_part || a.act != 0 || ((uintptr_t)a.amax_part & 7) || (a.amax_ld % 2) || a.amax_ld < 8 * cdiv(a.N, TB))) return false;
    if (a.ce) {
        if (a.ce < 1 || a.ce > 2 || conv || !a.out_f32 || a.resid || a.C2 || a.stats_out || a.amax_part || a.act != 0 || !a.ce_labels) return false;
        if (a.ce == 1 && (!a.lse_part || !a.ce_target)) return false;
        if (a.ce == 2 && (a.lse_part || !a.C || !a.ce_lse || !a.ce_g || (a.ldc % 8) != 0 || a.ldc < a.N || a.ldc > (long)TB * cdiv(a.N, TB))) return false;
    }
    if ((long)a.N * a.ldw * 2 >= (1l << 32)) return false;
    if (conv) {
        if ((a.Cin % BK) != 0 || a.Fout <= 0 || a.Tout <= 0) return false;
        if ((long)cdiv(a.M, (long)a.Fout * a.Tout) * a.Tin * a.Fin * a.Cin * 2 >= (1l << 32)) return false;
    } else if ((a.lda % 8) || (long)a.M * a.lda * 2 >= (1l << 32)) return false;
    return true;
}

template <typename K>
static bool set_lds_attr(K kernel, int bytes) { return ensure_dynamic_lds_ptr(reinterpret_cast<const void*>(kernel), (size_t)bytes); }

int gemm_8p_launch(const GemmArgs& a, bool conv, hipStream_t stream) {
    using kern_t = void (*)(GemmArgs);
    static const kern_t kerns[2][3] = {{gemm8p_kernel<false, 0>, gemm8p_kernel<false, 1>, gemm8p_kernel<false, 2>},
                                       {gemm8p_kernel<true, 0>, gemm8p_kernel<true, 1>, gemm8p_kernel<true, 2>}};
    if (a.act >= 0 && a.act <= 2 && !set_lds_attr(kerns[conv ? 1 : 0][a.act], 2 * BUF)) return MI_ERR_LAUNCH;
    if (a.act < 0 || a.act > 4) return MI_ERR_ARG;
    const int grid = cdiv(a.M, TB) * cdiv(a.N, TB);
    if (a.act >= 3) {
        const bool attr_t = set_lds_attr(gemm8p_kernel<false, 3>, 2 * BUF) && set_lds_attr(gemm8p_kernel<false, 4>, 2 * BUF);
        (void)attr_t;
        if (a.act == 3) launch_dense(PF_8P, gemm8p_kernel<false, 3>, dim3(grid), dim3(512), (size_t)2 * BUF, stream, a);
        else launch_dense(PF_8P_GELU, gemm8p_kernel<false, 4>, dim3(grid), dim3(512), (size_t)2 * BUF, stream, a);
        return MI_OK;
    }
    if (a.out_f32 && a.ce) {
        const kern_t kc = a.ce == 1 ? gemm8p_kernel<false, 0, true, false, false, false, false, 1> : gemm8p_kernel<false, 0, true, false, false, false, false, 2>;
        if (!set_lds_attr(kc, 2 * BUF)) return MI_ERR_LAUNCH;
        launch_dense(PF_8P_CE, kc, dim3(grid), dim3(512), (size_t)2 * BUF, stream, a);
        return MI_OK;
    }
    if (a.out_f32 && a.amax_part) {
        const bool attr_m = set_lds_attr(gemm8p_kernel<false, 0, true, false, false, false, true>, 2 * BUF);
        (void)attr_m;
        launch_dense(PF_8P_AMAX, gemm8p_kernel<false, 0, true, false, false, false, true>, dim3(grid), dim3(512), (size_t)2 * BUF, stream, a);
        return MI_OK;
    }
    if (a.out_f32 && a.lse_part) {
        const bool attr_e = set_lds_attr(gemm8p_kernel<false, 0, true, false, false, true>, 2 * BUF);
        (void)attr_e;
        launch_dense(PF_8P_OUT32, gemm8p_kernel<false, 0, true, false, false, true>, dim3(grid), dim3(512), (size_t)2 * BUF, stream, a);
        return MI_OK;
    }
    if (a.out_f32) {
        const bool attr32 = set_lds_attr(gemm8p_kernel<false, 0, true>, 2 * BUF);
        (void)attr32;
        launch_dense(PF_8P_OUT32, gemm8p_kernel<false, 0, true>, dim3(grid), dim3(512), (size_t)2 * BUF, stream, a);
        return MI_OK;
    }
    if (a.ln_stats) {
        const bool attr_l = set_lds_attr(gemm8p_kernel<false, 0, false, false, true>, 2 * BUF + 2048) && set_lds_attr(gemm8p_kernel<false, 1, false, false, true>, 2 * BUF + 2048);
        (void)attr_l;
        if (a.act) launch_dense(PF_8P_GELU, gemm8p_kernel<false, 1, false, false, true>, dim3(grid), dim3(512), (size_t)2 * BUF + 2048, stream, a);
        else launch_dense(PF_8P, gemm8p_kernel<false, 0, false, false, true>, dim3(grid), dim3(512), (size_t)2 * BUF + 2048, stream, a);
        return MI_OK;
    }
    if (a.gated) {
        const bool attr_g = set_lds_attr(gemm8p_kernel<true, 1, false, true>, 2 * BUF);
        (void)attr_g;
        launch_dense(PF_8P_CONV, gemm8p_kernel<true, 1, false, true>, dim3(grid), dim3(512), (size_t)2 * BUF, stream, a);
        return MI_OK;
    }
    launch_dense(conv ? PF_8P_CONV : (a.act ? PF_8P_GELU : PF_8P), kerns[conv ? 1 : 0][a.act], dim3(grid), dim3(512), (size_t)2 * BUF, stream, a);
    return MI_OK;
}

bool gemm_8p128_supported(const GemmArgs& a) {
    if (a.M <= 0 || a.N <= 0 || (a.N % 128) != 0 || (a.K % BK) != 0 || a.K < 5 * BK) return false;
    if (a.col_T || a.bias_mode == 2) return false;
    if (a.resid && !a.out_f32) return false;
    if (((uintptr_t)a.A & 15) || ((uintptr_t)a.W & 15) || ((uintptr_t)a.C & 15) || (a.lda % 8) || (a.ldw % 8)) return false;
    if (a.out_f32 ? (a.ldc % 4) != 0 : (a.ldc % 8) != 0) return false;
    if (a.resid && (((uintptr_t)a.resid & 15) || (a.ldr % 4) != 0)) return false;
    if (a.bias_mode == 1 && ((uintptr_t)a.bias & 15)) return false;
    if ((long)a.M * a.lda * 2 >= (1l << 32) || (long)a.N * a.ldw * 2 >= (1l << 32)) return false;
    if (a.ln_stats) return false;
    if ((a.C2 || a.stats_out) && (!a.out_f32 || a.N > 512 || (a.K % 128) != 0 || (a.C2 && (((uintptr_t)a.C2 & 7) || (a.ldc2 % 4))) || ((uintptr_t)a.stats_out & 7))) return false;
    return true;
}

int gemm_8p128_launch(const GemmArgs& a, int ring, hipStream_t stream) {
    const bool attr_set = set_lds_attr(gemm8p128_kernel<4>, 4 * B128_BUF);
    (void)attr_set;
    const int grid = cdiv(a.M, 128) * (a.N / 128);
    if (ring == 0) ring = (GEMM128_LOADER == 1 && a.K >= 2048) ? 2 : 3;
    if (ring == 2) {
        const bool attr_l = set_lds_attr(gemm8p128l_kernel, 4 * B128_BUF);
        (void)attr_l;
        launch_dense(PF_8P128, gemm8p128l_kernel, dim3(grid), dim3(512), (size_t)4 * B128_BUF, stream, a);
        return MI_OK;
    }
    if (ring == 3) {
        const bool attr_p = set_lds_attr(gemm8p128p_kernel, 4 * B128_BUF);
        (void)attr_p;
        launch_dense(PF_8P128, gemm8p128p_kernel, dim3(grid), dim3(512), (size_t)4 * B128_BUF, stream, a);
        return MI_OK;
    }
    launch_dense(PF_8P128, gemm8p128_kernel<4>, dim3(grid), dim3(512), (size_t)4 * B128_BUF, stream, a);
    return MI_OK;
}
```

huggingface_asr_amd/csrc/gemm_args.hpp:

```cpp
#pragma once
#include "common.hpp"
#include <hip/hip_ext.h>

struct GemmArgs {
    const bf16_t* A; long lda;
    const bf16_t* W; long ldw;
    const float* bias; int bias_mode;
    void* C; long ldc; int out_f32;
    const float* resid; long ldr; float alpha;
    int act;
    int col_T, col_Tp;
    int M, N, K;
    int variant;
    int Tin, Fin, Cin, Tout, Fout, KW, stride, pad_t, pad_f;
    int stride_f;
    int gated;
    const float* ln_stats; int ln_npart; const float* ln_colsum; float ln_eps;
    bf16_t* C2; long ldc2; float* stats_out;
    const bf16_t* aux; long ldaux; int aux_kind; float drop_p; unsigned long long drop_key;
    float* lse_part; int lse_ld;
    float* amax_part; int amax_ld;
    int ce; const long* ce_labels; float* ce_target; const float* ce_lse; const float* ce_g;
};
constexpr int LN_STATS_STRIDE = 32;

bool gemm_glds_supported(const GemmArgs& a, bool conv);
int gemm_glds_launch(const GemmArgs& a, bool conv, hipStream_t stream);


bool gemm_8p_supported(const GemmArgs& a, bool conv);
int gemm_8p_launch(const GemmArgs& a, bool conv, hipStream_t stream);
bool gemm_8p128_supported(const GemmArgs& a);
int gemm_8p128_launch(const GemmArgs& a, int ring, hipStream_t stream);


extern "C" int mi_profile_take_events(hipEvent_t* start, hipEvent_t* stop, int family);
enum { PF_8P = 0, PF_8P_GELU = 1, PF_8P_CONV = 2, PF_8P_OUT32 = 3, PF_8P128 = 4, PF_GLDS = 5, PF_GENERIC = 6, PF_8P_AMAX = 7, PF_8P_CE = 8, PF_COUNT = 9 };

template <typename F, typename... Args>
inline void launch_dense(int family, F kernel, dim3 grid, dim3 block, size_t lds, hipStream_t stream, Args... args) {
    hipEvent_t e0, e1;
    if (mi_profile_take_events(&e0, &e1, family)) hipExtLaunchKernelGGL(kernel, grid, block, (std::uint32_t)lds, stream, e0, e1, 0, args...);
    else hipLaunchKernelGGL(kernel, grid, block, lds, stream, args...);
}
```

huggingface_asr_amd/csrc/gemm_bf16.hip:

```cpp
#include "gemm_args.hpp"

namespace {

constexpr int BM = 128, BN = 128, BK = 64;
constexpr int NT = 256;

__device__ __forceinline__ int swz(int row, int chunk) { return chunk ^ ((row >> 1) & 7); }

template <bool CONV>
__global__ __launch_bounds__(NT) void gemm_bf16_kernel(GemmArgs p) {
    extern __shared__ __attribute__((aligned(16))) char smem[];
    bf16_t* sA = reinterpret_cast<bf16_t*>(smem);
    bf16_t* sB = sA + 2 * BM * BK;

    const int tid = threadIdx.x;
    const int lane = tid & 63, wave = tid >> 6;
    const int wm = wave >> 1, wn = wave & 1;

    const int ntm = (p.M + BM - 1) / BM, ntn = (p.N + BN - 1) / BN;
    const int nwg = ntm * ntn;
    int bid = blockIdx.x;
    {
        const int q = nwg >> 3, r = nwg & 7, xcd = bid & 7, idx = bid >> 3;
        bid = (xcd < r ? xcd * (q + 1) : r * (q + 1) + (xcd - r) * q) + idx;
// ... 142 lines not shown
        if (!conv || a.act != 1 || (a.N % 256) != 0 || !gemm_8p_supported(a, true)) return MI_ERR_UNSUPPORTED;
        const int slot = mi_profile_hook_begin(stream, 2.0 * a.M * a.N * a.K);
        const int rc = gemm_8p_launch(a, true, stream);
        if (slot >= 0) mi_profile_hook_end(slot, stream);
        if (rc != MI_OK) return rc;
        MI_CHECK_LAUNCH();
        return MI_OK;
    }
    if (gemm_glds_supported(a, conv)) {
        const int slot = mi_profile_hook_begin(stream, 2.0 * a.M * a.N * a.K);
        const int rc = gemm_glds_launch(a, conv, stream);
        if (slot >= 0) mi_profile_hook_end(slot, stream);
        if (rc != MI_OK) return rc;
        MI_CHECK_LAUNCH();
        return MI_OK;
    }
    const int grid = cdiv(a.M, BM) * cdiv(a.N, BN);
    const size_t lds = 2 * (BM + BN) * BK * sizeof(bf16_t);
    const int slot = mi_profile_hook_begin(stream, 2.0 * a.M * a.N * a.K);
    if (conv) launch_dense(PF_GENERIC, gemm_bf16_kernel<true>, dim3(grid), dim3(NT), lds, stream, a);
    else launch_dense(PF_GENERIC, gemm_bf16_kernel<false>, dim3(grid), dim3(NT), lds, stream, a);
    if (slot >= 0) mi_profile_hook_end(slot, stream);
    MI_CHECK_LAUNCH();
    return MI_OK;
}

}

extern "C" int mi_gemm_bf16_v(const void* A, long lda, const void* W, long ldw, const float* bias, int bias_mode,
                              void* C, long ldc, int out_f32, const float* resid, long ldr, float alpha, int act,
                              int M, int N, int K, int col_T, int col_Tp, int variant, hipStream_t stream) {
    MI_ENTER();
    GemmArgs a{};
    a.variant = variant;
    a.A = (const bf16_t*)A; a.lda = lda; a.W = (const bf16_t*)W; a.ldw = ldw;
    a.bias = bias; a.bias_mode = bias ? bias_mode : 0;
    a.C = C; a.ldc = ldc; a.out_f32 = out_f32; a.resid = resid; a.ldr = ldr; a.alpha = alpha; a.act = act;
    a.M = M; a.N = N; a.K = K; a.col_T = col_T; a.col_Tp = col_Tp;
    return launch(a, false, stream);
}
extern "C" int mi_gemm_bf16(const void* A, long lda, const void* W, long ldw, const float* bias, int bias_mode,
                            void* C, long ldc, int out_f32, const float* resid, long ldr, float alpha, int act,
                            int M, int N, int K, int col_T, int col_Tp, hipStream_t stream) {
    return mi_gemm_bf16_v(A, lda, W, ldw, bias, bias_mode, C, ldc, out_f32, resid, ldr, alpha, act, M, N, K, col_T, col_Tp, 0, stream);
}

extern "C" int mi_conv2d_cl_bf16_v(const void* in, const void* weight, const float* bias, void* out,
                                   int B, int Tin, int Fin, int Cin, int Cout, int KH, int KW, int stride,
                                   int pad_t, int pad_f, int Tout, int Fout, int act, int variant, hipStream_t stream) {
    MI_ENTER();
    GemmArgs a{};
    a.variant = variant;
    a.A = (const bf16_t*)in; a.lda = 0; a.W = (const bf16_t*)weight; a.ldw = (long)KH * KW * Cin;
    a.bias = bias; a.bias_mode = bias ? 1 : 0;
    a.C = out; a.ldc = Cout; a.out_f32 = 0; a.resid = nullptr; a.ldr = 0; a.alpha = 1.f; a.act = act;
    a.M = B * Tout * Fout; a.N = Cout; a.K = KH * KW * Cin;
    a.Tin = Tin; a.Fin = Fin; a.Cin = Cin; a.Tout = Tout; a.Fout = Fout; a.KW = KW; a.stride = stride; a.stride_f = stride;
    a.pad_t = pad_t; a.pad_f = pad_f;
    return launch(a, true, stream);
}
extern "C" int mi_conv2d_cl_bf16(const void* in, const void* weight, const float* bias, void* out,
                                 int B, int Tin, int Fin, int Cin, int Cout, int KH, int KW, int stride,
                                 int pad_t, int pad_f, int Tout, int Fout, int act, hipStream_t stream) {
    return mi_conv2d_cl_bf16_v(in, weight, bias, out, B, Tin, Fin, Cin, Cout, KH, KW, stride, pad_t, pad_f, Tout, Fout, act, 0, stream);
}

extern "C" int mi_conv2d_cl_geo_bf16(const void* in, const void* weight, const float* bias, void* out,
                                     int B, int Tin, int Fin, int Cin, int Cout, int KH, int KW, int stride_t, int stride_f,
                                     int pad_t, int pad_f, int Tout, int Fout, int act, int gated, hipStream_t stream) {
    MI_ENTER();
    if (stride_t <= 0 || stride_f <= 0 || KH <= 0 || KW <= 0 || Tout <= 0 || Fout <= 0) return MI_ERR_ARG;
    if ((long)(Tout - 1) * stride_t - pad_t >= Tin || (long)(Fout - 1) * stride_f - pad_f >= Fin) return MI_ERR_ARG;
    GemmArgs a{};
    const int Nw = gated ? 2 * Cout : Cout;
    a.A = (const bf16_t*)in; a.lda = 0; a.W = (const bf16_t*)weight; a.ldw = (long)KH * KW * Cin;
    a.bias = bias; a.bias_mode = bias ? 1 : 0;
    a.C = out; a.ldc = Cout; a.out_f32 = 0; a.resid = nullptr; a.ldr = 0; a.alpha = 1.f; a.act = act;
    a.M = B * Tout * Fout; a.N = Nw; a.K = KH * KW * Cin;
    a.Tin = Tin; a.Fin = Fin; a.Cin = Cin; a.Tout = Tout; a.Fout = Fout; a.KW = KW; a.stride = stride_t; a.stride_f = stride_f;
    a.pad_t = pad_t; a.pad_f = pad_f; a.gated = gated ? 1 : 0;
    return launch(a, true, stream);
}

extern "C" int mi_gemm_lnfold_bf16(const void* xb, long lda, const void* Wf, long ldw, const float* colsum, const float* cbias, const float* stats, int npart, float eps,
                                   void* C, long ldc, int act, int M, int N, int K, hipStream_t stream) {
    MI_ENTER();
    GemmArgs a{};
    a.A = (const bf16_t*)xb; a.lda = lda; a.W = (const bf16_t*)Wf; a.ldw = ldw; a.bias = cbias; a.bias_mode = 1;
    a.C = C; a.ldc = ldc; a.out_f32 = 0; a.alpha = 1.f; a.act = act; a.M = M; a.N = N; a.K = K;
    a.ln_stats = stats; a.ln_npart = npart; a.ln_colsum = colsum; a.ln_eps = eps;
    if (!xb || !Wf || !colsum || !cbias || !stats || !C || act < 0 || act > 1) return MI_ERR_ARG;
    if (!gemm_8p_supported(a, false)) return MI_ERR_UNSUPPORTED;
    const int slot = mi_profile_hook_begin(stream, 2.0 * M * N * K);
    const int rc = gemm_8p_launch(a, false, stream);
    if (slot >= 0) mi_profile_hook_end(slot, stream);
    if (rc != MI_OK) return rc;
    MI_CHECK_LAUNCH();
    return MI_OK;
}

extern "C" int mi_gemm_act_fwd_bf16(const void* A, long lda, const void* W, long ldw, const float* bias, void* pre, long ldp, void* h, long ldh, int kind,
                                    float drop_p, unsigned seed, unsigned stream_id, int M, int N, int K, hipStream_t stream) {
    MI_ENTER();
    GemmArgs a{};
    a.A = (const bf16_t*)A; a.lda = lda; a.W = (const bf16_t*)W; a.ldw = ldw; a.bias = bias; a.bias_mode = bias ? 1 : 0;
    a.C = pre; a.ldc = ldp; a.out_f32 = 0; a.alpha = 1.f; a.act = 4; a.M = M; a.N = N; a.K = K;
    a.C2 = (bf16_t*)h; a.ldc2 = ldh; a.aux_kind = kind; a.drop_p = drop_p; a.drop_key = ((unsigned long long)stream_id << 32) ^ (unsigned long long)seed;
    if (!A || !W || !pre || !h) return MI_ERR_ARG;
    if (!gemm_8p_supported(a, false)) return MI_ERR_UNSUPPORTED;
    const int slot = mi_profile_hook_begin(stream, 2.0 * M * N * K);
    const int rc = gemm_8p_launch(a, false, stream);
    if (slot >= 0) mi_profile_hook_end(slot, stream);
    if (rc != MI_OK) return rc;
    MI_CHECK_LAUNCH();
    return MI_OK;
}
extern "C" int mi_gemm_act_bwd_bf16(const void* dY, long ldy, const void* Wt, long ldw, const void* pre, long ldp, void* dX, long ldx, int kind,
                                    float drop_p, unsigned seed, unsigned stream_id, int M, int N, int K, hipStream_t stream) {
    MI_ENTER();
    GemmArgs a{};
    a.A = (const bf16_t*)dY; a.lda = ldy; a.W = (const bf16_t*)Wt; a.ldw = ldw; a.bias = nullptr; a.bias_mode = 0;
    a.C = dX; a.ldc = ldx; a.out_f32 = 0; a.alpha = 1.f; a.act = 3; a.M = M; a.N = N; a.K = K;
    a.aux = (const bf16_t*)pre; a.ldaux = ldp; a.aux_kind = kind; a.drop_p = drop_p; a.drop_key = ((unsigned long long)stream_id << 32) ^ (unsigned long long)seed;
    if (!dY || !Wt || !pre || !dX) return MI_ERR_ARG;
    if (!gemm_8p_supported(a, false)) return MI_ERR_UNSUPPORTED;
    const int slot = mi_profile_hook_begin(stream, 2.0 * M * N * K);
    const int rc = gemm_8p_launch(a, false, stream);
    if (slot >= 0) mi_profile_hook_end(slot, stream);
    if (rc != MI_OK) return rc;
    MI_CHECK_LAUNCH();
    return MI_OK;
}

extern "C" int mi_gemm_dropout_bf16(const void* A, long lda, const void* W, long ldw, const float* bias, void* C, long ldc, int out_f32, const float* resid, long ldr,
                                    float alpha, float drop_p, unsigned seed, unsigned stream_id, int M, int N, int K, hipStream_t stream) {
    MI_ENTER();
    GemmArgs a{};
    a.A = (const bf16_t*)A; a.lda = lda; a.W = (const bf16_t*)W; a.ldw = ldw; a.bias = bias; a.bias_mode = bias ? 1 : 0;
    a.C = C; a.ldc = ldc; a.out_f32 = out_f32; a.resid = resid; a.ldr = ldr; a.alpha = alpha; a.act = 0; a.M = M; a.N = N; a.K = K;
    a.drop_p = drop_p; a.drop_key = ((unsigned long long)stream_id << 32) ^ (unsigned long long)seed;
    if (!A || !W || !C || drop_p < 0.f || drop_p >= 1.f || (!out_f32 && (resid || alpha != 1.f))) return MI_ERR_ARG;
    if ((K % 128) != 0 || !gemm_8p128_supported(a)) return MI_ERR_UNSUPPORTED;
    const int slot = mi_profile_hook_begin(stream, 2.0 * M * N * K);
    const int rc = gemm_8p128_launch(a, 0, stream);
    if (slot >= 0) mi_profile_hook_end(slot, stream);
    if (rc != MI_OK) return rc;
    MI_CHECK_LAUNCH();
    return MI_OK;
}

extern "C" int mi_gemm_resid_stats_f32_v(const void* A, long lda, const void* W, long ldw, const float* bias, float* C, long ldc, const float* resid, long ldr, float alpha,
                                         void* C2, long ldc2, float* stats_out, int M, int N, int K, int variant, hipStream_t stream);
extern "C" int mi_gemm_resid_stats_f32(const void* A, long lda, const void* W, long ldw, const float* bias, float* C, long ldc, const float* resid, long ldr, float alpha,
                                       void* C2, long ldc2, float* stats_out, int M, int N, int K, hipStream_t stream) {
    return mi_gemm_resid_stats_f32_v(A, lda, W, ldw, bias, C, ldc, resid, ldr, alpha, C2, ldc2, stats_out, M, N, K, 0, stream);
}
extern "C" int mi_gemm_resid_stats_f32_v(const void* A, long lda, const void* W, long ldw, const float* bias, float* C, long ldc, const float* resid, long ldr, float alpha,
                                         void* C2, long ldc2, float* stats_out, int M, int N, int K, int variant, hipStream_t stream) {
    MI_ENTER();
    GemmArgs a{};
    a.A = (const bf16_t*)A; a.lda = lda; a.W = (const bf16_t*)W; a.ldw = ldw; a.bias = bias; a.bias_mode = bias ? 1 : 0;
    a.C = C; a.ldc = ldc; a.out_f32 = 1; a.resid = resid; a.ldr = ldr; a.alpha = alpha; a.act = 0; a.M = M; a.N = N; a.K = K;
    a.C2 = (bf16_t*)C2; a.ldc2 = ldc2; a.stats_out = stats_out;
    if (!A || !W || !C || !resid || (variant != 0 && variant != 40 && variant != 42 && variant != 43)) return MI_ERR_ARG;
    const bool wide = variant == 40;
    if (wide ? !gemm_8p_supported(a, false) : !gemm_8p128_supported(a)) return MI_ERR_UNSUPPORTED;
    const int slot = mi_profile_hook_begin(stream, 2.0 * M * N * K);
    const int rc = wide ? gemm_8p_launch(a, false, stream) : gemm_8p128_launch(a, variant == 42 ? 3 : (variant == 43 ? 2 : 0), stream);
    if (slot >= 0) mi_profile_hook_end(slot, stream);
    if (rc != MI_OK) return rc;
    MI_CHECK_LAUNCH();
    return MI_OK;
}

// ... 152 lines not shown
```

huggingface_asr_amd/ops.py:

```python
from __future__ import annotations

import math

import torch

from . import _lib

BF16 = torch.bfloat16


def _p(t):
    return 0 if t is None else t.data_ptr()


_PINNED_STREAM = None


def _stream():
    return torch.cuda.current_stream().cuda_stream if _PINNED_STREAM is None else _PINNED_STREAM


class pinned_stream:

    def __enter__(self):
# ... 35 lines not shown


def conv2d_first_gelu(x, w, bias, stride=2, pad=1, causal=False):
    B, T, F = x.shape
    Cc, KK = w.shape
    K = int(round(math.sqrt(KK)))
    T1, F1 = (T + 2 * pad - K) // stride + 1, (F + 2 * pad - K) // stride + 1
    out = torch.empty((B, T1, F1, Cc), device=x.device, dtype=BF16)
    pl = 2 * pad if causal else pad
    rc = _lib.lib().mi_conv2d_first_gelu(x.data_ptr(), w.data_ptr(), bias.data_ptr(), out.data_ptr(), B, T, F, Cc, K,
                                         stride, pl, pl, T1, F1, _stream())
    _lib.check(rc, "mi_conv2d_first_gelu")
    return out


def conv2d_cl(x, w, bias, K=3, stride=2, pad=1, causal=False, act="gelu", variant=0):
    B, T, F, Cin = x.shape
    Cout = w.shape[0]
    KH, KW = (K, K) if isinstance(K, int) else K
    pt, pf = (pad, pad) if isinstance(pad, int) else pad
    T1, F1 = (T + 2 * pt - KH) // stride + 1, (F + 2 * pf - KW) // stride + 1
    out = torch.empty((B, T1, F1, Cout), device=x.device, dtype=BF16)
    plt, plf = (2 * pt, 2 * pf) if causal else (pt, pf)
    rc = _lib.lib().mi_conv2d_cl_bf16_v(x.data_ptr(), w.data_ptr(), _p(bias), out.data_ptr(), B, T, F, Cin, Cout, KH, KW, stride,
                                        plt, plf, T1, F1, {"none": 0, "gelu": 1}[act], int(variant), _stream())
    _lib.check(rc, "mi_conv2d_cl_bf16")
    return out


def _geo_out(n, k, s, p):
    return (n + 2 * p - k) // s + 1


def conv2d_first_geo(x, w, bias, K=(3, 3), stride=(2, 2), pad=(1, 1), act="gelu"):
    B, T, F = x.shape
    Cc = w.shape[0]
    (KH, KW), (st, sf), (pt, pf) = K, stride, pad
    T1, F1 = _geo_out(T, KH, st, pt), _geo_out(F, KW, sf, pf)
    out = torch.empty((B, T1, F1, Cc), device=x.device, dtype=BF16)
    _lib.check(_lib.lib().mi_conv2d_first_geo(x.data_ptr(), w.data_ptr(), bias.data_ptr(), out.data_ptr(), B, T, F, Cc, KH, KW, st, sf, pt, pf, T1, F1,
                                              {"none": 0, "gelu": 1}[act], _stream()), "mi_conv2d_first_geo")
    return out


def conv2d_first_gated_gelu(x, w, bias, gw, gbias, stride=2, pad=1):
    B, T, F = x.shape
    Cc, KK = w.shape
    K = int(round(math.sqrt(KK)))
    T1, F1 = _geo_out(T, K, stride, pad), _geo_out(F, K, stride, pad)
    out = torch.empty((B, T1, F1, Cc), device=x.device, dtype=BF16)
    _lib.check(_lib.lib().mi_conv2d_first_gated_gelu(x.data_ptr(), w.data_ptr(), bias.data_ptr(), gw.data_ptr(), gbias.data_ptr(), out.data_ptr(), B, T, F, Cc, K,
                                                     stride, pad, pad, T1, F1, _stream()), "mi_conv2d_first_gated_gelu")
    return out


def conv2d_cl_geo(x, w, bias, K=(3, 3), stride=(2, 2), pad=(1, 1), act="gelu", gated=False):
    B, T, F, Cin = x.shape
    Cout = w.shape[0] // (2 if gated else 1)
    (KH, KW), (st, sf), (pt, pf) = K, stride, pad
    T1, F1 = _geo_out(T, KH, st, pt), _geo_out(F, KW, sf, pf)
    out = torch.empty((B, T1, F1, Cout), device=x.device, dtype=BF16)
    _lib.check(_lib.lib().mi_conv2d_cl_geo_bf16(x.data_ptr(), w.data_ptr(), _p(bias), out.data_ptr(), B, T, F, Cin, Cout, KH, KW, st, sf, pt, pf, T1, F1,
                                                {"none": 0, "gelu": 1}[act], int(gated), _stream()), "mi_conv2d_cl_geo_bf16")
    return out


def gated_act(z, g, B, T, Fq, C, share=1, blk=0, out=None):
    z2, g2 = z.reshape(-1, z.shape[-1]), g.reshape(-1, g.shape[-1])
    if out is None:
        out = torch.empty((B * T * Fq, C), device=z.device, dtype=BF16)
    _lib.check(_lib.lib().mi_gated_act_bf16(z2.data_ptr(), z2.stride(0), g2.data_ptr(), g2.stride(0), out.data_ptr(), out.stride(0), B, T, Fq, C, share, blk, _stream()),
               "mi_gated_act_bf16")
    return out


def gemm_lnfold(xb, wf, colsum, cbias, stats, npart, eps=1e-5, act="none", out=None):
    M, K = xb.shape
    N = wf.shape[0]
    if out is None:
        out = torch.empty((M, N), device=xb.device, dtype=BF16)
    _lib.check(_lib.lib().mi_gemm_lnfold_bf16(xb.data_ptr(), xb.stride(0), wf.data_ptr(), wf.stride(0), colsum.data_ptr(), cbias.data_ptr(), stats.data_ptr(), int(npart), float(eps),
                                              out.data_ptr(), out.stride(0), {"none": 0, "gelu": 1}[act], M, N, K, _stream()), "mi_gemm_lnfold_bf16")
    return out


def gemm_resid_stats(a, w, bias, resid, alpha=1.0, wide=False, variant=None):
    M, K = a.shape
    N = w.shape[0]
    c = torch.empty((M, N), device=a.device, dtype=torch.float32)
    c2 = torch.empty((M, N), device=a.device, dtype=BF16)
    st = torch.zeros((M, 32), device=a.device, dtype=torch.float32)
    _lib.check(_lib.lib().mi_gemm_resid_stats_f32_v(a.data_ptr(), a.stride(0), w.data_ptr(), w.stride(0), _p(bias), c.data_ptr(), c.stride(0), _p(resid), resid.stride(0) if resid is not None else 0,
                                                    float(alpha), c2.data_ptr(), c2.stride(0), st.data_ptr(), M, N, K, (40 if wide else 0) if variant is None else int(variant), _stream()), "mi_gemm_resid_stats_f32_v")
    return c, c2, st


def layernorm_fold(x, ln=None, eps=1e-5, lengths=None, T=1):
    M, d = x.shape
    g, b = ln if ln else (None, None)
    y = torch.empty_like(x)
    yb = torch.empty((M, d), device=x.device, dtype=BF16)
    st = torch.zeros((M, 32), device=x.device, dtype=torch.float32)
    _lib.check(_lib.lib().mi_layernorm_fold(x.data_ptr(), x.stride(0), _p(lengths), T, _p(g), _p(b), float(eps), y.data_ptr(), y.stride(0), yb.data_ptr(), yb.stride(0), st.data_ptr(),
                                            M, d, _stream()), "mi_layernorm_fold")
    return y, yb, st


def layernorm_chain(x, *, lengths=None, T=1, ln1=None, eps1=1e-5, store_y=None, lna=None, eps2=1e-5, outa=None,
                    outa32=None, lnb=None, outb=None):
    M, d = x.shape
    g1, b1 = ln1 if ln1 else (None, None)
    ga, ba = lna if lna else (None, None)
    gb, bb = lnb if lnb else (None, None)
    rc = _lib.lib().mi_layernorm_chain(x.data_ptr(), x.stride(0), _p(lengths), T, _p(g1), _p(b1), eps1,
                                       _p(store_y), store_y.stride(0) if store_y is not None else 0,
                                       _p(ga), _p(ba), eps2, _p(outa), outa.stride(0) if outa is not None else 0,
                                       _p(outa32), outa32.stride(0) if outa32 is not None else 0,
                                       _p(gb), _p(bb), _p(outb), outb.stride(0) if outb is not None else 0, M, d, _stream())
    _lib.check(rc, "mi_layernorm_chain")


def rotary(x, cos, sin, T, H):
    M, d = x.shape
    out = torch.empty_like(x)
    rc = _lib.lib().mi_rotary_bf16(x.data_ptr(), x.stride(0), out.data_ptr(), out.stride(0), cos.data_ptr(), sin.data_ptr(),
                                   M, T, H, d // H, _stream())
    _lib.check(rc, "mi_rotary_bf16")
    return out


def attention(q, k, vt, Tp, B, T, H, *, pos=None, bias_u=None, bias_v=None, lengths=None, causal=False):
    d = vt.shape[0]
    hd = d // H
    out = torch.empty((B * T, d), device=q.device, dtype=BF16)
    rc = _lib.lib().mi_attention_bf16(q.data_ptr(), q.stride(0), k.data_ptr(), k.stride(0), vt.data_ptr(), vt.stride(0), Tp,
                                      _p(pos), pos.stride(0) if pos is not None else 0, _p(bias_u), _p(bias_v), _p(lengths),
                                      out.data_ptr(), out.stride(0), B, T, H, hd, 1.0 / math.sqrt(hd), int(causal), _stream())
    _lib.check(rc, "mi_attention_bf16")
    return out


def attention_qkv(qkv, B, T, H, *, pos=None, bias_u=None, bias_v=None, lengths=None, causal=False, lse=None, drop=None, variant=0):
    d = qkv.shape[1] // 3
    hd = d // H
    out = torch.empty((B * T, d), device=qkv.device, dtype=BF16)
    q, k, v = qkv[:, :d], qkv[:, d:2 * d], qkv[:, 2 * d:]
    operands = (q.data_ptr(), qkv.stride(0), k.data_ptr(), qkv.stride(0), v.data_ptr(), qkv.stride(0),
               _p(pos), pos.stride(0) if pos is not None else 0, _p(bias_u), _p(bias_v), _p(lengths), out.data_ptr(), out.stride(0))
    if lse is not None:
        dp, dseed, dsid = drop if drop is not None else (0.0, 0, 0)
        rc = _lib.lib().mi_attention_qkv_lse_bf16(*operands, lse.data_ptr(), B, T, H, hd, 1.0 / math.sqrt(hd), int(causal),
                                                  float(dp), int(dseed) & 0xFFFFFFFF, int(dsid) & 0xFFFFFFFF, _stream())
        _lib.check(rc, "mi_attention_qkv_lse_bf16")
        return out
    rc = _lib.lib().mi_attention_qkv_bf16_v(*operands, B, T, 0, 0, H, hd, 1.0 / math.sqrt(hd), int(causal), int(variant), _stream())
    _lib.check(rc, "mi_attention_qkv_bf16_v")
    return out


def attention_general(q, k, v, B, Tq, Tk, H, *, lengths=None, causal=False, out=None, kv_bstride=0, variant=0):
    d = q.shape[1]
    hd = d // H
    if out is None:
        out = torch.empty((B * Tq, d), device=q.device, dtype=BF16)
    rc = _lib.lib().mi_attention_qkv_bf16_v(q.data_ptr(), q.stride(0), k.data_ptr(), k.stride(0), v.data_ptr(), v.stride(0),
                                            0, 0, 0, 0, _p(lengths), out.data_ptr(), out.stride(0), B, Tq, Tk, kv_bstride, H, hd,
                                            1.0 / math.sqrt(hd), int(causal), int(variant), _stream())
    _lib.check(rc, "mi_attention_qkv_bf16_v")
    return out


def row_stats(x, eps=1e-5):
    M, d = x.shape
    st = torch.empty((M, 2), device=x.device, dtype=torch.float32)
    rc = _lib.lib().mi_row_stats_bf16(x.data_ptr(), x.stride(0), d, eps, st.data_ptr(), M, _stream())
    _lib.check(rc, "mi_row_stats_bf16")
    return st


def csgu(u, gamma, beta, w, bias, B, T, *, pad_left=None, dilation=1, act=0, eps=1e-5, stats=None):
    M, C2 = u.shape
    Cc = C2 // 2
    K = w.shape[-1]
    st = row_stats(u[:, Cc:], eps) if stats is None else stats
    out = torch.empty((M, Cc), device=u.device, dtype=BF16)
    rc = _lib.lib().mi_csgu_bf16(u.data_ptr(), u.stride(0), st.data_ptr(), gamma.data_ptr(), beta.data_ptr(), w.data_ptr(),
                                 _p(bias), out.data_ptr(), out.stride(0), B, T, Cc, K,
                                 (K - 1) // 2 if pad_left is None else pad_left, dilation, act, _stream())
    _lib.check(rc, "mi_csgu_bf16")
    return out


def csgu_conv(u, stats, gamma, beta, w, bias, B, T, *, pad_left=None, dilation=1):
    M, C2 = u.shape
    Cc = C2 // 2
    K = w.shape[-1]
    out = torch.empty((M, Cc), device=u.device, dtype=BF16)
    rc = _lib.lib().mi_csgu_conv_bf16(u.data_ptr(), u.stride(0), stats.data_ptr(), gamma.data_ptr(), beta.data_ptr(), w.data_ptr(), _p(bias),
                                      out.data_ptr(), out.stride(0), B, T, Cc, K, (K - 1) // 2 if pad_left is None else int(pad_left), int(dilation), _stream())
    _lib.check(rc, "mi_csgu_conv_bf16")
    return out


def gate_act_mul(r, g, act=0):
    M, Cc = g.shape
    out = torch.empty((M, Cc), device=g.device, dtype=BF16)
    rc = _lib.lib().mi_gate_act_mul_bf16(r.data_ptr(), r.stride(0), g.data_ptr(), g.stride(0), out.data_ptr(), out.stride(0), M, Cc, int(act), _stream())
    _lib.check(rc, "mi_gate_act_mul_bf16")
    return out


def dwconv_residual(m, w, bias, B, T, pad_left=None):
    M, Cc = m.shape
    K = w.shape[-1]
    out = torch.empty_like(m)
    rc = _lib.lib().mi_dwconv_residual_bf16(m.data_ptr(), m.stride(0), w.data_ptr(), _p(bias), out.data_ptr(), out.stride(0),
                                            B, T, Cc, K, (K - 1) // 2 if pad_left is None else int(pad_left), _stream())
    _lib.check(rc, "mi_dwconv_residual_bf16")
    return out


def gemm_lse(a, w, bias, out):
    _req(a, BF16); _req(w, BF16)
    M, K = a.shape
    N = w.shape[0]
    L = _lib.lib()
    lse = torch.empty((M,), device=a.device, dtype=torch.float32)
    ws = torch.empty((int(L.mi_gemm_lse_workspace_floats(M, N)),), device=a.device, dtype=torch.float32)
    rc = L.mi_gemm_lse_f32(a.data_ptr(), a.stride(0), w.data_ptr(), w.stride(0), _p(bias), out.data_ptr(), out.stride(0), lse.data_ptr(), ws.data_ptr(), M, N, K, _stream())
    if rc == _lib.ERR_UNSUPPORTED:
        gemm(a, w, bias, out=out)
        return row_lse(out[:, :N])
    _lib.check(rc, "mi_gemm_lse_f32")
    return lse


def linear_rows(x, w, bias=None, *, act="none", out=None, out_dtype=BF16, accumulate=False, kv_cache=None, U=1, past=0):
    _req(x, BF16); _req(w, BF16)
    M, K = x.shape
    N = w.shape[0]
    if out is None:
        out = torch.empty((M, N), device=x.device, dtype=out_dtype)
    L = _lib.lib()
    nbytes = L.mi_linear_rows_workspace_bytes(M, N, K)
    ws = torch.empty(max(nbytes, 1), dtype=torch.uint8, device=x.device)
    f32 = out.dtype == torch.float32
    kc, vc = kv_cache if kv_cache is not None else (None, None)
    rc = L.mi_linear_rows(x.data_ptr(), x.stride(0), w.data_ptr(), w.stride(0), _p(bias), {"none": 0, "gelu": 1, "gelu_new": 2}[act],
                          out.data_ptr() if f32 else None, out.stride(0) if f32 else 0, int(bool(accumulate)), None if f32 else out.data_ptr(), 0 if f32 else out.stride(0),
                          _p(kc), _p(vc), int(U), int(past), kc.shape[1] if kc is not None else 0, kc.shape[2] if kc is not None else 0, M, N, K,
                          ws.data_ptr(), nbytes, _stream())
    _lib.check(rc, "mi_linear_rows")
    return out


def row_lse(x):
    M, V = x.shape
    out = torch.empty((M,), device=x.device, dtype=torch.float32)
    rc = _lib.lib().mi_row_lse(x.data_ptr(), x.stride(0), 0 if x.dtype == torch.float32 else 1, V, out.data_ptr(), M, _stream())
    _lib.check(rc, "mi_row_lse")
    return out


def row_argmax(x):
    _req(x)
    if x.dtype not in (torch.float32, BF16) or x.dim() != 2 or x.stride(1) != 1:
        raise TypeError("row_argmax: a 2-D fp32 / bf16 tensor with contiguous rows")
    M, V = x.shape
    out = torch.empty((M,), device=x.device, dtype=torch.int32)
    rc = _lib.lib().mi_row_argmax(x.data_ptr(), x.stride(0), 0 if x.dtype == torch.float32 else 1, V, out.data_ptr(), M, _stream())
    _lib.check(rc, "mi_row_argmax")
    return out
# ... 505 lines not shown
```

include/hfasr_hip.h:

```cpp
#ifndef HFASR_HIP_H
#define HFASR_HIP_H
#include <stddef.h>
#include <stdint.h>

#ifdef __cplusplus
extern "C" {
#endif

typedef struct ihipStream_t* mi_stream_t;

const char* mi_last_error(void);

int mi_profile_create(int capacity);
void mi_profile_enable(int on);
void mi_profile_reset(void);
int mi_profile_count(void);
int mi_profile_summary(double* total_ms, double* total_flops);
int mi_profile_calibrate(mi_stream_t stream, int n, double* median_ms);
int mi_profile_summary_family(int family, double* total_ms, double* total_flops, int* launches);

int mi_gemm_bf16(const void* A, long lda, const void* W, long ldw, const float* bias, int bias_mode,
                 void* C, long ldc, int out_f32, const float* resid, long ldr, float alpha, int act,
                 int M, int N, int K, int col_T, int col_Tp, mi_stream_t stream);
int mi_gemm_bf16_v(const void* A, long lda, const void* W, long ldw, const float* bias, int bias_mode,
                   void* C, long ldc, int out_f32, const float* resid, long ldr, float alpha, int act,
                   int M, int N, int K, int col_T, int col_Tp, int variant, mi_stream_t stream);

int mi_conv2d_cl_bf16(const void* in, const void* weight, const float* bias, void* out,
                      int B, int Tin, int Fin, int Cin, int Cout, int KH, int KW, int stride,
                      int pad_t, int pad_f, int Tout, int Fout, int act, mi_stream_t stream);
int mi_conv2d_cl_bf16_v(const void* in, const void* weight, const float* bias, void* out,
                        int B, int Tin, int Fin, int Cin, int Cout, int KH, int KW, int stride,
                        int pad_t, int pad_f, int Tout, int Fout, int act, int variant, mi_stream_t stream);

int mi_conv2d_first_gelu(const float* x, const float* w, const float* bias, void* out_cl_bf16,
                         int B, int T, int F, int C, int K, int stride, int pad_t, int pad_f,
                         int T1, int F1, mi_stream_t stream);

int mi_conv2d_first_geo(const float* x, const float* w, const float* bias, void* out_cl_bf16, int B, int T, int F, int C,
                        int KH, int KW, int stride_t, int stride_f, int pad_t, int pad_f, int T1, int F1, int act, mi_stream_t stream);
int mi_conv2d_first_gated_gelu(const float* x, const float* w, const float* bias, const float* gw, const float* gbias, void* out_cl_bf16,
                               int B, int T, int F, int C, int K, int stride, int pad_t, int pad_f, int T1, int F1, mi_stream_t stream);
int mi_conv2d_cl_geo_bf16(const void* in, const void* weight, const float* bias, void* out, int B, int Tin, int Fin, int Cin, int Cout, int KH, int KW,
                          int stride_t, int stride_f, int pad_t, int pad_f, int Tout, int Fout, int act, int gated, mi_stream_t stream);
int mi_gated_act_bf16(const void* z, long ldz, const void* g, long ldg, void* out, long ldo, int B, int T, int Fq, int C, int share, int blk, mi_stream_t stream);

int mi_gemm_dropout_bf16(const void* A, long lda, const void* W, long ldw, const float* bias, void* C, long ldc, int out_f32, const float* resid, long ldr,
                         float alpha, float drop_p, unsigned seed, unsigned stream_id, int M, int N, int K, mi_stream_t stream);
int mi_gemm_act_fwd_bf16(const void* A, long lda, const void* W, long ldw, const float* bias, void* pre, long ldp, void* h, long ldh, int kind,
                         float drop_p, unsigned seed, unsigned stream_id, int M, int N, int K, mi_stream_t stream);
int mi_gemm_act_bwd_bf16(const void* dY, long ldy, const void* Wt, long ldw, const void* pre, long ldp, void* dX, long ldx, int kind,
                         float drop_p, unsigned seed, unsigned stream_id, int M, int N, int K, mi_stream_t stream);
int mi_gemm_lnfold_bf16(const void* xb, long lda, const void* Wf, long ldw, const float* colsum, const float* cbias, const float* stats, int npart, float eps,
                        void* C, long ldc, int act, int M, int N, int K, mi_stream_t stream);
int mi_gemm_resid_stats_f32(const void* A, long lda, const void* W, long ldw, const float* bias, float* C, long ldc, const float* resid, long ldr, float alpha,
                            void* C2, long ldc2, float* stats_out, int M, int N, int K, mi_stream_t stream);
int mi_gemm_resid_stats_f32_v(const void* A, long lda, const void* W, long ldw, const float* bias, float* C, long ldc, const float* resid, long ldr, float alpha,
                              void* C2, long ldc2, float* stats_out, int M, int N, int K, int variant, mi_stream_t stream);
int mi_layernorm_fold(const float* x, long ldx, const int* lengths, int T, const float* g1, const float* b1, float eps1, float* y32, long ldy,
                      void* yb_bf16, long ldyb, float* stats, int M, int d, mi_stream_t stream);

int mi_layernorm_chain(const float* x, long ldx, const int* lengths, int T,
                       const float* g1, const float* b1, float eps1, float* y32, long ldy,
                       const float* ga, const float* ba, float eps2, void* outa_bf16, long lda,
                       float* outa_f32, long lda32,
                       const float* gb, const float* bb, void* outb_bf16, long ldb,
                       int M, int d, mi_stream_t stream);

int mi_cast_f32_bf16(const float* x, long ldx, void* out, long ldo, int M, int d, mi_stream_t stream);

int mi_rotary_bf16(const void* x, long ldx, void* out, long ldo, const float* cos_t, const float* sin_t,
                   int M, int T, int H, int hd, mi_stream_t stream);

int mi_attention_bf16(const void* q, long ldq, const void* k, long ldk, const void* vt, long ldvt, int Tp,
                      const void* pos, long ldp, const float* bias_u, const float* bias_v,
                      const int* lengths, void* out, long ldo, int B, int T, int H, int hd,
                      float scale, int causal, mi_stream_t stream);

int mi_attention_qkv_bf16(const void* q, long ldq, const void* k, long ldk, const void* v, long ldv,
                          const void* pos, long ldp, const float* bias_u, const float* bias_v,
                          const int* lengths, void* out, long ldo, int B, int T, int Tk, long kv_bstride, int H, int hd,
                          float scale, int causal, mi_stream_t stream);
int mi_attention_qkv_bf16_v(const void* q, long ldq, const void* k, long ldk, const void* v, long ldv,
                            const void* pos, long ldp, const float* bias_u, const float* bias_v,
                            const int* lengths, void* out, long ldo, int B, int T, int Tk, long kv_bstride, int H, int hd,
                            float scale, int causal, int variant, mi_stream_t stream);

int mi_attention_qkv_lse_bf16(const void* q, long ldq, const void* k, long ldk, const void* v, long ldv,
                              const void* pos, long ldp, const float* bias_u, const float* bias_v,
                              const int* lengths, void* out, long ldo, float* lse, int B, int T, int H, int hd,
                              float scale, int causal, float drop_p, unsigned seed, unsigned stream_id, mi_stream_t stream);
int mi_attention_qkv_bwd_probs(const void* q, long ldq, const void* k, long ldk, const void* v, long ldv,
                               const void* pos, long ldp, const float* bias_u, const float* bias_v, const int* lengths,
                               const void* ctx, long ldo, const void* dctx, long ldd, const float* lse,
                               void* prob, void* ds, long ldsr, void* dbd, long ldbd, int pad,
                               void* dq, long lddq, float* dsum_u, float* dsum_v, void* qu_out, void* qv_out, long ldqb,
                               int B, int T, int H, int hd, float scale, int causal, float drop_p, unsigned seed, unsigned stream_id, int flags, mi_stream_t stream);
int mi_attention_qkv_bwd_fused(const void* q, const void* k, const void* v, long ldqkv, const int* lengths,
                               const void* ctx, long ldo, const void* dctx, long ldd, const float* lse,
                               void* dq, void* dk, void* dv, long ldg, void* workspace, size_t ws_bytes,
                               int B, int T, int H, int hd, float scale, mi_stream_t stream);
int mi_attention_x_lse_bf16(const void* q, long ldq, const void* k, long ldk, const void* v, long ldv, const int* lengths, void* out, long ldo, float* lse,
                            int B, int Tq, int Tk, int H, int hd, float scale, int causal, float drop_p, unsigned seed, unsigned stream_id, mi_stream_t stream);
int mi_attention_x_bwd_probs(const void* q, long ldq, const void* k, long ldk, const void* v, long ldv, const int* lengths, const void* ctx, long ldo,
                             const void* dctx, long ldd, const float* lse, void* prob, void* ds, long ldsr, void* dq, long lddq,
                             int B, int Tq, int Tk, int H, int hd, float scale, int causal, float drop_p, unsigned seed, unsigned stream_id, mi_stream_t stream);

int mi_row_stats_bf16(const void* x, long ldx, int d, float eps, float* stats, int M, mi_stream_t stream);
int mi_csgu_bf16(const void* u, long ldu, const float* stats, const float* gamma, const float* beta,
                 const float* w, const float* bias, void* out, long ldo,
                 int B, int T, int C, int K, int pad_left, int dilation, int act, mi_stream_t stream);

int mi_dwconv_residual_bf16(const void* m, long ldm, const float* w, const float* bias, void* out, long ldo,
                            int B, int T, int C, int K, int pad_left, mi_stream_t stream);
int mi_csgu_conv_bf16(const void* u, long ldu, const float* stats, const float* gamma, const float* beta, const float* w, const float* bias,
                      void* out, long ldo, int B, int T, int C, int K, int pad_left, int dilation, mi_stream_t stream);
int mi_gate_act_mul_bf16(const void* r, long ldr, const void* g, long ldg, void* out, long ldo, long M, int C, int act, mi_stream_t stream);
int mi_gate_act_mul_bwd_bf16(const void* r, long ldr, const void* g, long ldg, const void* ds, long ldds, void* dr, long lddr, void* dg, long lddg,
                             long M, int C, int act, mi_stream_t stream);

int mi_fbank_f64(const float* wave, long ldw, const int* num_samples, int N, const double* window,
                 const double* twiddle, const double* mel_t, const int* mel_lo, const int* mel_hi,
                 float* out, int T_out, int B, int nmel, double mel_floor, double preemph, mi_stream_t stream);
int mi_trim_zeros_pad_f32(const float* wave, long ldw, const int* num_samples, int N, int B, int min_len, float* out, long ldo, int N_out,
                          int* first, int* valid, int* eff_len, mi_stream_t stream);
int mi_cmvn_utterance(float* x, const int* frames, int B, int T, int nmel, int norm_means, int norm_vars,
                      float pad, mi_stream_t stream);
int mi_cmvn_global(float* x, long total, int nmel, const float* means, const float* stds, mi_stream_t stream);

int mi_row_lse(const void* x, long ld, int dtype, int V, float* lse, int M, mi_stream_t stream);
size_t mi_gemm_lse_workspace_floats(int M, int N);
int mi_gemm_lse_f32(const void* A, long lda, const void* W, long ldw, const float* bias, float* C, long ldc, float* lse, float* workspace,
                    int M, int N, int K, mi_stream_t stream);
int mi_row_argmax(const void* x, long ld, int dtype, int V1, int* best, int M, mi_stream_t stream);
int mi_ctc_collapse(const int* best, int B, int T, const int* lengths, int blank, long pad_id, void* tokens, int tokens_dtype, int* n_tokens, int* frames,
                    mi_stream_t stream);
int mi_ctc_greedy(const void* logits, long ld_row, long ld_batch, int dtype, int B, int T, int V1, const int* lengths, int blank, long pad_id,
                  int* best, void* tokens, int tokens_dtype, int* n_tokens, int* frames, mi_stream_t stream);

size_t mi_ctc_beam_workspace_bytes(int B, int T, int W);
int mi_ctc_beam_cut(const void* logits, long ld_row, long ld_batch, int dtype, int B, int T, int V1, const int* lengths, int blank, int K, float* lse, float* lp_blank,
                    float* cut_lp, int* cut_id, mi_stream_t stream);
int mi_ctc_beam_walk(const void* logits, long ld_row, long ld_batch, int dtype, int B, int T, int V1, const int* lengths, int blank, long pad_id, int W, int K, int nbest,
                     const float* lse, const float* lp_blank, const float* cut_lp, const int* cut_id, void* workspace, size_t workspace_bytes, void* tokens,
                     int tokens_dtype, int* n_tokens, float* scores, int* frames, mi_stream_t stream);
size_t mi_ctc_beam_stream_state_bytes(int B, int max_frames, int W);
int mi_ctc_beam_stream_reset(void* state, size_t state_bytes, int B, int max_frames, int W, mi_stream_t stream);
int mi_ctc_beam_stream_walk(const void* logits, long ld_row, long ld_batch, int dtype, int B, int T_call, int V1, const int* n_valid, int blank, long pad_id, int W, int K,
                            int nbest, const float* lse, const float* lp_blank, const float* cut_lp, const int* cut_id, void* state, size_t state_bytes, int max_frames,
                            int final, int* committed, int* committed_frames, int* n_committed, int* n_new, void* tokens, int tokens_dtype, int* n_tokens,
                            float* scores, int* frames, mi_stream_t stream);
size_t mi_ctc_align_workspace_bytes(int B, int T, int U);
int mi_ctc_align(const void* logits, long ld_b, long ld_t, int dtype, const float* lse, int T, const long* labels, int U, const int* in_len, int blank, int V1, int B,
                 void* workspace, size_t workspace_bytes, int* path, float* score, int* tgt_len, int* start, int* end, float* token_lp, mi_stream_t stream);
size_t mi_gemm_argmax_workspace_floats(int M, int N);
int mi_gemm_argmax_bf16(const void* A, long lda, const void* W, long ldw, const float* bias, int* best, float* workspace, int M, int N, int K, mi_stream_t stream);
int mi_gemm_ce_f32(const void* A, long lda, const void* W, long ldw, const float* bias, const long* labels, float* acc, float* lse, float* nll, float* target,
                   float* workspace, int M, int N, int K, mi_stream_t stream);
int mi_gemm_ce_bwd_bf16(const void* A, long lda, const void* W, long ldw, const float* bias, const long* labels, const float* lse, const float* g,
                        void* dlogits, long ldo, int M, int N, int K, mi_stream_t stream);
int mi_ctc_loss_fwd(const void* logits, long ld_b, long ld_t, int dtype, const float* lse, int T,
                    const long* labels, int U, const int* in_len, int blank, int B,
                    int reduction, int zero_infinity, float* nll, int* tgt_len, float* loss, mi_stream_t stream);

int mi_ctc_prefix_prepare(const void* logits, long ld_b, long ld_t, int dtype, const int* lens, int B, int T, int O,
                          int blank, int W, float* lse_scratch, float* x_out, float* r0_out, mi_stream_t stream);
int mi_ctc_prefix_score(const float* x, int B, int T, int O, int blank, int W, const float* r_prev, const long* last_ids,
                        long ld_last, int out_len, const float* s_prev, float* psi_out, float* scores_out, mi_stream_t stream);
int mi_ctc_prefix_advance(const float* x, int B, int T, int O, int blank, int W, const float* r_old, const long* last_old, long ld_last_old, int out_len_old,
                          const float* psi_old, const long* last, long ld_last, int out_len, float* r_prev, float* psi, float* scores, mi_stream_t stream);
int mi_ctc_prefix_score_full(const float* x, int B, int T, int O, int blank, int W, const float* r_prev, int rp_full, const float* psi_old, const long* last,
                             long ld_last, int out_len, float* r_all, float* psi, float* scores, mi_stream_t stream);

int mi_embed_tokens(const long* ids, const float* wte, float scale, const float* pos, int pos_offset, int U, int d,
                    int M, int V, float* out, mi_stream_t stream);
int mi_ce_label_smoothing(const float* logits, long ld, const long* labels, int B, int U, int shift, int V, float eps,
                          float* acc, float* row_loss, mi_stream_t stream);

int mi_transpose_bf16(const void* in, long ld_in, void* out, long ld_out, int M, int N, int Mp, mi_stream_t stream);
int mi_transpose_many_bf16(const void* descs, int count, mi_stream_t stream);
size_t mi_colsum_workspace_floats(int M, int N);
int mi_colsum(const void* x, long ld, int dtype, int M, int N, float* out, float* workspace, mi_stream_t stream);
int mi_colsum_cast_bf16(const float* x, long ld, int M, int N, void* out, mi_stream_t stream);
int mi_colsum2_acc_f32(const float* a, const float* b, long ld, int M, int N, float* out_a, float* out_b, mi_stream_t stream);
int mi_act_fwd_bf16(const void* pre, long ldp, void* out, long ldo, int M, int N, int kind, mi_stream_t stream);
int mi_act_bwd_bf16(const void* dy, long lddy, const void* pre, long ldp, void* dx, long lddx, int M, int N, int kind,
                    mi_stream_t stream);
int mi_act_dropout_fwd_bf16(const void* pre, long ldp, void* out, long ldo, int M, int N, int kind, float p, unsigned seed, unsigned stream_id,
                            mi_stream_t stream);
int mi_act_dropout_bwd_bf16(const void* dy, long lddy, const void* pre, long ldp, void* dx, long lddx, int M, int N, int kind, float p,
                            unsigned seed, unsigned stream_id, mi_stream_t stream);
size_t mi_layernorm_bwd_workspace_floats(int d);
int mi_layernorm_bwd(const void* x, long ldx, int x_bf16, const float* gamma, float eps, const void* dy, long lddy, int dy_f32,
                     void* dx, long lddx, int dx_bf16, int accumulate, float* dgamma, float* dbeta, float* workspace, int M, int d,
// ... 261 lines not shown
```

Baseline: 83180 audio-seconds/sec.

## Fuse CSGU layernorm row statistics into the MLP up-projection GEMM epilogue

The MLP up-projection GEMM now emits per-row partial sum and sum-of-squares over the gate half of its output, computed with MFMA against a ones vector in the epilogue. The CSGU depthwise-conv kernel reduces these partials into mean and rstd itself, so the separate row_stats pass that re-read the gate half is dropped. The cost is extra MFMAs and LDS in the GEMM epilogue, plus variance computed as E[x^2]-mean^2, which is less numerically robust than the two-pass form.

```diff
diff --git a/huggingface_asr_amd/_lib.py b/huggingface_asr_amd/_lib.py
--- a/huggingface_asr_amd/_lib.py
+++ b/huggingface_asr_amd/_lib.py
@@ -41,6 +41,9 @@
     "mi_gated_act_bwd_bf16": [vp, i64, vp, i64, vp, i64, vp, i64, vp, i64, i32, i32, i32, i32, i32, vp],
     "mi_conv2d_first_wgrad": [vp, vp, vp, vp] + [i32] * 12 + [vp, vp],
     "mi_gemm_lnfold_bf16": [vp, i64, vp, i64, vp, vp, vp, i32, f32, vp, i64, i32, i32, i32, i32, vp],
+    "mi_gemm_lnfold_stats_bf16": [vp, i64, vp, i64, vp, vp, vp, i32, f32, vp, i64, i32, vp, i32, i32, i32, i32, i32, i32, vp],
+    "mi_gemm_stats_bf16": [vp, i64, vp, i64, vp, vp, i64, i32, vp, i32, i32, i32, i32, i32, i32, vp],
+    "mi_csgu_partials_bf16": [vp, i64, vp, i32, i32, f32, vp, vp, vp, vp, vp, i64, i32, i32, i32, i32, i32, i32, i32, vp],
     "mi_gemm_resid_stats_f32": [vp, i64, vp, i64, vp, vp, i64, vp, i64, f32, vp, i64, vp, i32, i32, i32, vp],
     "mi_layernorm_fold": [vp, i64, vp, i32, vp, vp, f32, vp, i64, vp, i64, vp, i32, i32, vp],
     "mi_layernorm_chain": [vp, i64, vp, i32, vp, vp, f32, vp, i64, vp, vp, f32, vp, i64, vp, i64, vp, vp, vp, i64, i32, i32, vp],
diff --git a/huggingface_asr_amd/csrc/conv.hip b/huggingface_asr_amd/csrc/conv.hip
--- a/huggingface_asr_amd/csrc/conv.hip
+++ b/huggingface_asr_amd/csrc/conv.hip
@@ -271,6 +271,7 @@
     const bf16_t* in; long ld_in;
     const bf16_t* mul; long ld_mul;
     const float* stats;
+    const float* part; int part_ld, npart; float eps;
     const float* gamma; const float* beta;
     const float* w; const float* bias;
     bf16_t* out; long ld_out;
@@ -331,7 +332,7 @@
 constexpr int DWF_K = 31, DWF_TT = 64, DWF_CT = 64, DWF_ROWS = DWF_TT + DWF_K - 1, DWF_PER = DWF_TT / 4;
 constexpr int DWF_WS = DWF_CT + 1, DWF_WBUF = (DWF_K * DWF_WS + 3) / 4 * 4;
 
-template <bool CSGU>
+template <bool CSGU, bool PART = false>
 __global__ __launch_bounds__(256) void dwconv31_kernel(DwArgs p) {
     extern __shared__ __attribute__((aligned(16))) char smem[];
     float* tile = reinterpret_cast<float*>(smem);
@@ -347,6 +348,7 @@
     const int ch = tid & 7;
     bf16x8 vin[NPI], vio[NPO];
     float mu[NPI], rs[NPI];
+    f32x4 pa[NPI], pb[NPI];
     bool ok[NPI];
 #pragma unroll
     for (int q = 0; q < NPI; ++q) {
@@ -356,7 +358,10 @@
         const long row = (long)b * p.T + min(max(t, 0), p.T - 1);
         vin[q] = *reinterpret_cast<const bf16x8*>(p.in + row * p.ld_in + c0 + ch * 8);
         mu[q] = 0.f; rs[q] = 0.f;
-        if (CSGU) { mu[q] = p.stats[2 * row]; rs[q] = p.stats[2 * row + 1]; }
+        if constexpr (PART) {
+            const f32x4* pr = reinterpret_cast<const f32x4*>(p.part + row * p.part_ld);
+            pa[q] = pr[0]; pb[q] = pr[p.npart > 2 ? 1 : 0];
+        } else if (CSGU) { mu[q] = p.stats[2 * row]; rs[q] = p.stats[2 * row + 1]; }
     }
     f32x4 g0 = {1.f, 1.f, 1.f, 1.f}, g1 = g0, b0 = {0.f, 0.f, 0.f, 0.f}, b1 = b0;
     if (CSGU) {
@@ -369,6 +374,17 @@
         }
     }
     __builtin_amdgcn_sched_barrier(0);
+    if constexpr (PART) {
+        const bool h1 = p.npart > 1, h2 = p.npart > 2, h3 = p.npart > 3;
+        const float inv = 1.f / (float)p.C;
+#pragma unroll
+        for (int q = 0; q < NPI; ++q) {
+            const float sm = (pa[q].x + (h1 ? pa[q].z : 0.f)) + ((h2 ? pb[q].x : 0.f) + (h3 ? pb[q].z : 0.f));
+            const float sq = (pa[q].y + (h1 ? pa[q].w : 0.f)) + ((h2 ? pb[q].y : 0.f) + (h3 ? pb[q].w : 0.f));
+            mu[q] = sm * inv;
+            rs[q] = rsqrtf(fmaxf(sq * inv - mu[q] * mu[q], 0.f) + p.eps);
+        }
+    }
 #pragma unroll
     for (int q = 0; q < NPW; ++q) {
         const int i = tid + q * 256;
@@ -534,11 +550,13 @@
     if (fast) {
         dim3 gridf(a.C / DWF_CT, cdiv(a.T, DWF_TT), a.B);
         const size_t ldsf = (size_t)(DWF_ROWS * DWF_CT + DWF_WBUF) * sizeof(float) + (size_t)DWF_TT * DWF_CT * sizeof(bf16_t);
-        if (csgu) hipLaunchKernelGGL(dwconv31_kernel<true>, gridf, dim3(256), ldsf, stream, a);
+        if (csgu && a.part) hipLaunchKernelGGL((dwconv31_kernel<true, true>), gridf, dim3(256), ldsf, stream, a);
+        else if (csgu) hipLaunchKernelGGL(dwconv31_kernel<true>, gridf, dim3(256), ldsf, stream, a);
         else hipLaunchKernelGGL(dwconv31_kernel<false>, gridf, dim3(256), ldsf, stream, a);
         MI_CHECK_LAUNCH();
         return MI_OK;
     }
+    if (a.part) return MI_ERR_UNSUPPORTED;
     dim3 grid(cdiv(a.C, DW_CT), cdiv(a.T, DW_TT), a.B);
     if (csgu) hipLaunchKernelGGL(dwconv_time_kernel<true>, grid, dim3(256), lds, stream, a);
     else hipLaunchKernelGGL(dwconv_time_kernel<false>, grid, dim3(256), lds, stream, a);
@@ -552,6 +570,18 @@
     MI_ENTER();
     DwArgs a{};
     a.in = (const bf16_t*)u + C; a.ld_in = ldu; a.mul = (const bf16_t*)u; a.ld_mul = ldu; a.stats = stats;
+    a.gamma = gamma; a.beta = beta; a.w = w; a.bias = bias; a.out = (bf16_t*)out; a.ld_out = ldo;
+    a.B = B; a.T = T; a.C = C; a.K = K; a.pad_left = pad_left; a.dilation = dilation; a.act = act;
+    return dw_launch(a, true, stream);
+}
+
+extern "C" int mi_csgu_partials_bf16(const void* u, long ldu, const float* part, int part_ld, int npart, float eps, const float* gamma, const float* beta,
+                                     const float* w, const float* bias, void* out, long ldo,
+                                     int B, int T, int C, int K, int pad_left, int dilation, int act, hipStream_t stream) {
+    MI_ENTER();
+    if (!part || npart < 1 || npart > 4 || ((uintptr_t)part & 15) || (part_ld % 4) != 0 || part_ld < (npart > 2 ? 8 : 4)) return MI_ERR_ARG;
+    DwArgs a{};
+    a.in = (const bf16_t*)u + C; a.ld_in = ldu; a.mul = (const bf16_t*)u; a.ld_mul = ldu; a.part = part; a.part_ld = part_ld; a.npart = npart; a.eps = eps;
     a.gamma = gamma; a.beta = beta; a.w = w; a.bias = bias; a.out = (bf16_t*)out; a.ld_out = ldo;
     a.B = B; a.T = T; a.C = C; a.K = K; a.pad_left = pad_left; a.dilation = dilation; a.act = act;
     return dw_launch(a, true, stream);
diff --git a/huggingface_asr_amd/csrc/encoder.hip b/huggingface_asr_amd/csrc/encoder.hip
--- a/huggingface_asr_amd/csrc/encoder.hip
+++ b/huggingface_asr_amd/csrc/encoder.hip
@@ -7,6 +7,7 @@
     bf16_t *cv, *lin;
     bf16_t *z1, *g1, *z2, *g2;
     float *feo, *x, *stats, *lnst;
+    float *cgst;
     float *mixed, *lh, *sw;
     int* lens;
     size_t bytes;
@@ -38,6 +39,7 @@
     w.hid = bf(M * dd);
     w.stats = f32(M * 2);
     w.lnst = c.ln_fold ? f32(M * 32) : nullptr;
+    w.cgst = (c.ln_fold && dd >= 16) ? reinterpret_cast<float*>(w.a1) : nullptr;
     w.lens = (int*)k.take((size_t)2 * c.B * 4);
     w.mixed = w.lh = w.sw = nullptr;
     if (c.layer_mixing) { w.mixed = f32(M * dd); w.sw = f32((size_t)(c.L + 1)); }
@@ -71,6 +73,7 @@
     return true;
 }
 
+constexpr int CGST_LD = 8;
 constexpr float LEPS = 1e-5f;
 
 struct Fwd : Slots {
@@ -95,7 +98,7 @@
     int enter_layer(const float* src, int l) const;
     int project_positions(int layers) const;
     int attention_qkv(int l) const;
-    int local_gate(int l, hipStream_t sl) const;
+    int local_gate(int l, hipStream_t sl, const float* part = nullptr) const;
     int merge_dwconv(int l) const;
     int plain_layer(int l, int Lt) const;
     int folded_layer(int l) const;
@@ -167,8 +170,12 @@
                                  mask_len, w.ctx, d, c.B, T2, 0, 0, c.H, D.hd, scale, c.is_causal, st);
 }
 
-int Fwd::local_gate(int l, hipStream_t sl) const {
+int Fwd::local_gate(int l, hipStream_t sl, const float* part) const {
     const int kc = c.csgu_kernel;
+    if (part && !c.csgu_linear) {
+        const int rc = mi_csgu_partials_bf16(w.h, I, part, CGST_LD, I / 512, LEPS, Lf(l, CSGU_LN_G), Lf(l, CSGU_LN_B), Lf(l, CSGU_W), Lf(l, CSGU_B), w.s, I / 2, c.B, T2, I / 2, kc, cpad, dil, c.csgu_act, sl);
+        if (rc != MI_ERR_UNSUPPORTED) return rc;
+    }
     RUN(mi_row_stats_bf16(w.h + I / 2, I, I / 2, LEPS, w.stats, M, sl));
     if (!c.csgu_linear)
         return mi_csgu_bf16(w.h, I, w.stats, Lf(l, CSGU_LN_G), Lf(l, CSGU_LN_B), Lf(l, CSGU_W), Lf(l, CSGU_B), w.s, I / 2, c.B, T2, I / 2, kc, cpad, dil, c.csgu_act, sl);
@@ -247,8 +254,9 @@
     RUN(mi_gemm_lnfold_bf16(w.a0, d, Lw(l, QKV_WF), d, Lf(l, QKV_SF), Lf(l, QKV_CF), w.lnst, npg, LEPS, w.qk, 3 * d, 0, M, 3 * d, d, st));
     RUN(attention_qkv(l));
     RUN(mi_gemm_bf16_v(w.ctx, d, Lw(l, ATT_WO), d, Lf(l, ATT_BO), 1, w.cat, 2 * d, 0, nullptr, 0, 1.f, 0, M, d, d, 0, 0, gv, st));
-    RUN(mi_gemm_lnfold_bf16(w.a0, d, Lw(l, MLP_WF), d, Lf(l, MLP_SF), Lf(l, MLP_CF), w.lnst, npg, LEPS, w.h, I, 1, M, I, d, st));
-    RUN(local_gate(l, st));
+    float* gst = ((I / 2) % 256 == 0 && I / 512 <= 4 && ((uintptr_t)w.cgst & 15) == 0) ? w.cgst : nullptr;
+    RUN(mi_gemm_lnfold_stats_bf16(w.a0, d, Lw(l, MLP_WF), d, Lf(l, MLP_SF), Lf(l, MLP_CF), w.lnst, npg, LEPS, w.h, I, 1, gst, CGST_LD, I / 2, I, M, I, d, st));
+    RUN(local_gate(l, st, gst));
     RUN(mi_gemm_bf16_v(w.s, I / 2, Lw(l, MLP_W2), I / 2, Lf(l, MLP_B2), 1, w.cat + d, 2 * d, 0, nullptr, 0, 1.f, 0, M, d, I / 2, 0, 0, gv, st));
     RUN(merge_dwconv(l));
     RUN(mi_gemm_resid_stats_f32_v(w.m2, 2 * d, Lw(l, MRG_W), 2 * d, Lf(l, MRG_B), w.x, d, w.x, d, 1.0f, w.a0, d, w.lnst, M, d, 2 * d, gv, st));
diff --git a/huggingface_asr_amd/csrc/gemm_8p.hip b/huggingface_asr_amd/csrc/gemm_8p.hip
--- a/huggingface_asr_amd/csrc/gemm_8p.hip
+++ b/huggingface_asr_amd/csrc/gemm_8p.hip
@@ -15,6 +15,7 @@
 
 constexpr int TB = 256, BK = 64;
 constexpr int BUF = 65536, BOFF = 32768;
+constexpr int STAT_TABLE = 8192;
 
 template <int N>
 __device__ __forceinline__ void wait_vm() {
@@ -40,7 +41,7 @@
     unsigned aRd[2], bRd[2];
 };
 
-template <bool CONV, int ACT, bool OUT32 = false, bool GATED = false, bool LNF = false, bool LSE = false, bool AMAX = false, int CE = 0>
+template <bool CONV, int ACT, bool OUT32 = false, bool GATED = false, bool LNF = false, bool LSE = false, bool AMAX = false, int CE = 0, bool STATS = false>
 __global__ __launch_bounds__(512, 2) void gemm8p_kernel(GemmArgs p) {
     extern __shared__ __attribute__((aligned(16))) char smem[];
     const int tid = threadIdx.x, lane = tid & 63;
@@ -469,6 +470,10 @@
         }
         return;
     }
+    const bool st_tile = STATS && n0 >= p.stat_n0 && n0 < p.stat_n1;
+    bf16x8 st_ones;
+#pragma unroll
+    for (int e = 0; e < 8; ++e) st_ones[e] = (bf16_t)1.0f;
 #pragma unroll
     for (int blk = 0; blk < 4; ++blk) {
 #pragma unroll
@@ -491,6 +496,33 @@
             const uint4 v = *reinterpret_cast<const uint4*>(reg + row * 128 + ((pc ^ ((row >> 1) & 7)) << 4));
             const int m = m0 + wr * 128 + row;
             if (m < p.M) *reinterpret_cast<uint4*>(C + (long)m * p.ldc + nb + pc * 8) = v;
+        }
+        if constexpr (STATS) {
+            if (st_tile) {
+#pragma unroll
+                for (int ii = 0; ii < 2; ++ii) {
+                    const int row = (blk * 2 + ii) * 16 + fr;
+                    const bf16x8 h0 = *reinterpret_cast<const bf16x8*>(reg + row * 128 + ((fq ^ swz) << 4));
+                    const bf16x8 h1 = *reinterpret_cast<const bf16x8*>(reg + row * 128 + (((fq + 4) ^ swz) << 4));
+                    f32x4 sm = __builtin_amdgcn_mfma_f32_16x16x32_bf16(st_ones, h0, f32x4{0.f, 0.f, 0.f, 0.f}, 0, 0, 0);
+                    f32x4 sq = __builtin_amdgcn_mfma_f32_16x16x32_bf16(h0, h0, f32x4{0.f, 0.f, 0.f, 0.f}, 0, 0, 0);
+                    sm = __builtin_amdgcn_mfma_f32_16x16x32_bf16(st_ones, h1, sm, 0, 0, 0);
+                    sq = __builtin_amdgcn_mfma_f32_16x16x32_bf16(h1, h1, sq, 0, 0, 0);
+                    const float qd = (fr & 2) ? ((fr & 1) ? sq.w : sq.z) : ((fr & 1) ? sq.y : sq.x);
+                    if (fq == (fr >> 2)) *reinterpret_cast<f32x2*>(smem + 2 * BUF + 2048 + ((wr * 128 + row) * 4 + wc) * 8) = f32x2{sm.x, qd};
+                }
+            }
+        }
+    }
+    if constexpr (STATS) {
+        if (st_tile) {
+            asm volatile("s_waitcnt lgkmcnt(0)" ::: "memory");
+            barrier();
+            if (tid < TB) {
+                const f32x4 a = *reinterpret_cast<const f32x4*>(smem + 2 * BUF + 2048 + tid * 32), b = *reinterpret_cast<const f32x4*>(smem + 2 * BUF + 2048 + tid * 32 + 16);
+                if (m0 + tid < p.M)
+                    *reinterpret_cast<f32x2*>(p.stats_out + (long)(m0 + tid) * p.stat_ld + ((n0 - p.stat_n0) >> 8) * 2) = f32x2{(a.x + a.z) + (b.x + b.z), (a.y + a.w) + (b.y + b.w)};
+            }
         }
     }
 }
@@ -1095,6 +1127,10 @@
         if (conv || a.out_f32 || a.gated || a.ln_stats || a.resid || a.col_T || a.act > 4 || (a.aux_kind != 1 && a.aux_kind != 2) || a.drop_p < 0.f || a.drop_p >= 1.f) return false;
         if (a.act == 3 && (!a.aux || ((uintptr_t)a.aux & 15) || (a.ldaux % 8))) return false;
         if (a.act == 4 && (!a.C2 || ((uintptr_t)a.C2 & 15) || (a.ldc2 % 8))) return false;
+    } else if (a.stats_out && !a.out_f32) {
+        if (conv || a.gated || a.C2 || a.resid || a.act > 1 || ((uintptr_t)a.stats_out & 7)) return false;
+        if (a.stat_n0 < 0 || a.stat_n1 <= a.stat_n0 || a.stat_n1 > a.N || (a.stat_n0 % TB) != 0 || (a.stat_n1 % TB) != 0 || (a.stat_n1 - a.stat_n0) / TB > LN_STATS_STRIDE / 2) return false;
+        if ((a.stat_ld % 2) != 0 || a.stat_ld < 2 * ((a.stat_n1 - a.stat_n0) / TB)) return false;
     } else if (a.C2 || a.stats_out) {
         if (!a.out_f32 || !a.resid || a.N > 1024 || (a.C2 && (((uintptr_t)a.C2 & 7) || (a.ldc2 % 4))) || ((uintptr_t)a.stats_out & 7)) return false;
     }
@@ -1154,6 +1190,13 @@
         launch_dense(PF_8P_OUT32, gemm8p_kernel<false, 0, true>, dim3(grid), dim3(512), (size_t)2 * BUF, stream, a);
         return MI_OK;
     }
+    if (a.stats_out) {
+        const kern_t ks = a.ln_stats ? (a.act ? gemm8p_kernel<false, 1, false, false, true, false, false, 0, true> : gemm8p_kernel<false, 0, false, false, true, false, false, 0, true>)
+                                     : (a.act ? gemm8p_kernel<false, 1, false, false, false, false, false, 0, true> : gemm8p_kernel<false, 0, false, false, false, false, false, 0, true>);
+        if (!set_lds_attr(ks, 2 * BUF + 2048 + STAT_TABLE)) return MI_ERR_LAUNCH;
+        launch_dense(a.act ? PF_8P_GELU : PF_8P, ks, dim3(grid), dim3(512), (size_t)2 * BUF + 2048 + STAT_TABLE, stream, a);
+        return MI_OK;
+    }
     if (a.ln_stats) {
         const bool attr_l = set_lds_attr(gemm8p_kernel<false, 0, false, false, true>, 2 * BUF + 2048) && set_lds_attr(gemm8p_kernel<false, 1, false, false, true>, 2 * BUF + 2048);
         (void)attr_l;
diff --git a/huggingface_asr_amd/csrc/gemm_args.hpp b/huggingface_asr_amd/csrc/gemm_args.hpp
--- a/huggingface_asr_amd/csrc/gemm_args.hpp
+++ b/huggingface_asr_amd/csrc/gemm_args.hpp
@@ -21,6 +21,7 @@
     float* lse_part; int lse_ld;
     float* amax_part; int amax_ld;
     int ce; const long* ce_labels; float* ce_target; const float* ce_lse; const float* ce_g;
+    int stat_n0, stat_n1, stat_ld;
 };
 constexpr int LN_STATS_STRIDE = 32;
 
diff --git a/huggingface_asr_amd/csrc/gemm_bf16.hip b/huggingface_asr_amd/csrc/gemm_bf16.hip
--- a/huggingface_asr_amd/csrc/gemm_bf16.hip
+++ b/huggingface_asr_amd/csrc/gemm_bf16.hip
@@ -248,14 +248,36 @@
     return launch(a, true, stream);
 }
 
-extern "C" int mi_gemm_lnfold_bf16(const void* xb, long lda, const void* Wf, long ldw, const float* colsum, const float* cbias, const float* stats, int npart, float eps,
-                                   void* C, long ldc, int act, int M, int N, int K, hipStream_t stream) {
+extern "C" int mi_gemm_lnfold_stats_bf16(const void* xb, long lda, const void* Wf, long ldw, const float* colsum, const float* cbias, const float* stats, int npart, float eps,
+                                         void* C, long ldc, int act, float* stats_out, int stat_ld, int stat_n0, int stat_n1, int M, int N, int K, hipStream_t stream) {
     MI_ENTER();
     GemmArgs a{};
     a.A = (const bf16_t*)xb; a.lda = lda; a.W = (const bf16_t*)Wf; a.ldw = ldw; a.bias = cbias; a.bias_mode = 1;
     a.C = C; a.ldc = ldc; a.out_f32 = 0; a.alpha = 1.f; a.act = act; a.M = M; a.N = N; a.K = K;
     a.ln_stats = stats; a.ln_npart = npart; a.ln_colsum = colsum; a.ln_eps = eps;
+    a.stats_out = stats_out; a.stat_ld = stat_ld; a.stat_n0 = stats_out ? stat_n0 : 0; a.stat_n1 = stats_out ? stat_n1 : 0;
     if (!xb || !Wf || !colsum || !cbias || !stats || !C || act < 0 || act > 1) return MI_ERR_ARG;
+    if (!gemm_8p_supported(a, false)) return MI_ERR_UNSUPPORTED;
+    const int slot = mi_profile_hook_begin(stream, 2.0 * M * N * K);
+    const int rc = gemm_8p_launch(a, false, stream);
+    if (slot >= 0) mi_profile_hook_end(slot, stream);
+    if (rc != MI_OK) return rc;
+    MI_CHECK_LAUNCH();
+    return MI_OK;
+}
+extern "C" int mi_gemm_lnfold_bf16(const void* xb, long lda, const void* Wf, long ldw, const float* colsum, const float* cbias, const float* stats, int npart, float eps,
+                                   void* C, long ldc, int act, int M, int N, int K, hipStream_t stream) {
+    return mi_gemm_lnfold_stats_bf16(xb, lda, Wf, ldw, colsum, cbias, stats, npart, eps, C, ldc, act, nullptr, 0, 0, 0, M, N, K, stream);
+}
+
+extern "C" int mi_gemm_stats_bf16(const void* A, long lda, const void* W, long ldw, const float* bias, void* C, long ldc, int act, float* stats_out, int stat_ld, int stat_n0, int stat_n1,
+                                  int M, int N, int K, hipStream_t stream) {
+    MI_ENTER();
+    GemmArgs a{};
+    a.A = (const bf16_t*)A; a.lda = lda; a.W = (const bf16_t*)W; a.ldw = ldw; a.bias = bias; a.bias_mode = bias ? 1 : 0;
+    a.C = C; a.ldc = ldc; a.out_f32 = 0; a.alpha = 1.f; a.act = act; a.M = M; a.N = N; a.K = K;
+    a.stats_out = stats_out; a.stat_ld = stat_ld; a.stat_n0 = stat_n0; a.stat_n1 = stat_n1;
+    if (!A || !W || !C || !stats_out || act < 0 || act > 1) return MI_ERR_ARG;
     if (!gemm_8p_supported(a, false)) return MI_ERR_UNSUPPORTED;
     const int slot = mi_profile_hook_begin(stream, 2.0 * M * N * K);
     const int rc = gemm_8p_launch(a, false, stream);
diff --git a/huggingface_asr_amd/ops.py b/huggingface_asr_amd/ops.py
--- a/huggingface_asr_amd/ops.py
+++ b/huggingface_asr_amd/ops.py
@@ -141,6 +141,25 @@
     _lib.check(_lib.lib().mi_gemm_lnfold_bf16(xb.data_ptr(), xb.stride(0), wf.data_ptr(), wf.stride(0), colsum.data_ptr(), cbias.data_ptr(), stats.data_ptr(), int(npart), float(eps),
                                               out.data_ptr(), out.stride(0), {"none": 0, "gelu": 1}[act], M, N, K, _stream()), "mi_gemm_lnfold_bf16")
     return out
+
+
+def gemm_stats(a, w, bias, stat_range, act="none", out=None, stats_out=None, lnfold=None):
+    M, K = a.shape
+    N = w.shape[0]
+    if out is None:
+        out = torch.empty((M, N), device=a.device, dtype=BF16)
+    if stats_out is None:
+        stats_out = torch.zeros((M, 32), device=a.device, dtype=torch.float32)
+    n0, n1 = (int(v) for v in stat_range)
+    ac = {"none": 0, "gelu": 1}[act]
+    if lnfold is None:
+        _lib.check(_lib.lib().mi_gemm_stats_bf16(a.data_ptr(), a.stride(0), w.data_ptr(), w.stride(0), _p(bias), out.data_ptr(), out.stride(0), ac, stats_out.data_ptr(), stats_out.stride(0), n0, n1,
+                                                 M, N, K, _stream()), "mi_gemm_stats_bf16")
+    else:
+        colsum, stats, npart, eps = lnfold
+        _lib.check(_lib.lib().mi_gemm_lnfold_stats_bf16(a.data_ptr(), a.stride(0), w.data_ptr(), w.stride(0), colsum.data_ptr(), bias.data_ptr(), stats.data_ptr(), int(npart), float(eps),
+                                                        out.data_ptr(), out.stride(0), ac, stats_out.data_ptr(), stats_out.stride(0), n0, n1, M, N, K, _stream()), "mi_gemm_lnfold_stats_bf16")
+    return out, stats_out
 
 
 def gemm_resid_stats(a, w, bias, resid, alpha=1.0, wide=False, variant=None):
@@ -247,6 +266,17 @@
                                  _p(bias), out.data_ptr(), out.stride(0), B, T, Cc, K,
                                  (K - 1) // 2 if pad_left is None else pad_left, dilation, act, _stream())
     _lib.check(rc, "mi_csgu_bf16")
+    return out
+
+
+def csgu_partials(u, part, npart, gamma, beta, w, bias, B, T, *, act=0, eps=1e-5):
+    M, C2 = u.shape
+    Cc = C2 // 2
+    K = w.shape[-1]
+    out = torch.empty((M, Cc), device=u.device, dtype=BF16)
+    rc = _lib.lib().mi_csgu_partials_bf16(u.data_ptr(), u.stride(0), part.data_ptr(), part.stride(0), int(npart), float(eps), gamma.data_ptr(), beta.data_ptr(), w.data_ptr(),
+                                          _p(bias), out.data_ptr(), out.stride(0), B, T, Cc, K, (K - 1) // 2, 1, act, _stream())
+    _lib.check(rc, "mi_csgu_partials_bf16")
     return out
 
 
diff --git a/include/hfasr_hip.h b/include/hfasr_hip.h
--- a/include/hfasr_hip.h
+++ b/include/hfasr_hip.h
@@ -53,6 +53,10 @@
                          float drop_p, unsigned seed, unsigned stream_id, int M, int N, int K, mi_stream_t stream);
 int mi_gemm_lnfold_bf16(const void* xb, long lda, const void* Wf, long ldw, const float* colsum, const float* cbias, const float* stats, int npart, float eps,
                         void* C, long ldc, int act, int M, int N, int K, mi_stream_t stream);
+int mi_gemm_lnfold_stats_bf16(const void* xb, long lda, const void* Wf, long ldw, const float* colsum, const float* cbias, const float* stats, int npart, float eps,
+                              void* C, long ldc, int act, float* stats_out, int stat_ld, int stat_n0, int stat_n1, int M, int N, int K, mi_stream_t stream);
+int mi_gemm_stats_bf16(const void* A, long lda, const void* W, long ldw, const float* bias, void* C, long ldc, int act, float* stats_out, int stat_ld, int stat_n0, int stat_n1,
+                       int M, int N, int K, mi_stream_t stream);
 int mi_gemm_resid_stats_f32(const void* A, long lda, const void* W, long ldw, const float* bias, float* C, long ldc, const float* resid, long ldr, float alpha,
                             void* C2, long ldc2, float* stats_out, int M, int N, int K, mi_stream_t stream);
 int mi_gemm_resid_stats_f32_v(const void* A, long lda, const void* W, long ldw, const float* bias, float* C, long ldc, const float* resid, long ldr, float alpha,
@@ -110,6 +114,9 @@
 int mi_csgu_bf16(const void* u, long ldu, const float* stats, const float* gamma, const float* beta,
                  const float* w, const float* bias, void* out, long ldo,
                  int B, int T, int C, int K, int pad_left, int dilation, int act, mi_stream_t stream);
+int mi_csgu_partials_bf16(const void* u, long ldu, const float* part, int part_ld, int npart, float eps, const float* gamma, const float* beta,
+                          const float* w, const float* bias, void* out, long ldo,
+                          int B, int T, int C, int K, int pad_left, int dilation, int act, mi_stream_t stream);
 
 int mi_dwconv_residual_bf16(const void* m, long ldm, const float* w, const float* bias, void* out, long ldo,
                             int B, int T, int C, int K, int pad_left, mi_stream_t stream);
```

Result: no change. 83690 audio-seconds/sec (median of 6 runs) (+0.6%).
